# PSeitz/veloci

Hardware: AMD Instinct MI355X
Metric: queries/sec, 3-term AND on 100M-doc index (p50 latency and HBM fraction alongside) (higher is better)
Workload: dtype u32 doc ids + f16->f32 scores

## Files before the change

### veloci_amd/csrc/capi.cpp

```cpp
#include <chrono>
#include <thread>
#include <cstdio>
#include <cstdlib>
#include <cstring>

#include "../../include/veloci_amd.h"
#include <functional>
#include <future>

#include <dlfcn.h>
#include <unistd.h>

#include "engine.hpp"
#include "text.hpp"

using namespace vq;
using vqreq::Request;
using vqreq::VelociError;

namespace {
thread_local std::string g_err;

int fail(int code, const std::string& msg) {
    g_err = msg;
// ... 60 lines not shown
        for (size_t i = 0; i < kv.second.size(); ++i) {
            if (i) s += ',';
            vqjson::escape_to(s, kv.second[i]);
        }
        s += ']';
    }
    s += '}';
}

static void why_found_info_json(std::string& s, const Result& R) {
    s += '{';
    bool first = true;
    for (auto& [anchor, fields] : R.why_found_info) {
        if (!first) s += ',';
        first = false;
        s += '"' + std::to_string(anchor) + "\":";
        why_found_terms_json(s, fields);
    }
    s += '}';
}

namespace {
void dump_f32(std::string& s, float f) {
    uint32_t b;
    std::memcpy(&b, &f, 4);
    s += std::to_string(b);
}
template <class T, class F>
void dump_opt(std::string& s, const std::optional<T>& v, F f) {
    if (v) f(s, *v);
    else s += "null";
}
void dump_usize(std::string& s, size_t v) { s += std::to_string(v); }
void dump_bool(std::string& s, bool v) { s += v ? "true" : "false"; }
void dump_str(std::string& s, const std::string& v) { vqjson::escape_to(s, v); }
void dump_boost_part(std::string& s, const vqreq::RequestBoostPart& b) {
    static const char* const names[] = {"Log2", "Log10", "Multiply", "Add", "Replace"};
    s += "{\"path\":";
    dump_str(s, b.path);
    s += ",\"boost_fun\":";
    if (b.boost_fun) s += std::string("\"") + names[int(*b.boost_fun)] + "\"";
    else s += "null";
    s += ",\"param\":";
    dump_opt(s, b.param, dump_f32);
    s += ",\"skip_when_score\":";
    if (b.skip_when_score) {
        s += '[';
        for (size_t i = 0; i < b.skip_when_score->size(); ++i) {
            if (i) s += ',';
            dump_f32(s, (*b.skip_when_score)[i]);
        }
        s += ']';
    } else s += "null";
    s += ",\"expression\":";
    dump_opt(s, b.expression, dump_str);
    s += '}';
}
void dump_boost_list(std::string& s, const std::optional<std::vector<vqreq::RequestBoostPart>>& v) {
    if (!v) {
        s += "null";
        return;
    }
    s += '[';
    for (size_t i = 0; i < v->size(); ++i) {
        if (i) s += ',';
        dump_boost_part(s, (*v)[i]);
    }
    s += ']';
}
void dump_options(std::string& s, const std::optional<vqreq::SearchRequestOptions>& o) {
    if (!o) {
        s += "null";
        return;
    }
    s += "{\"explain\":";
    dump_bool(s, o->explain);
    s += ",\"top\":";
    dump_opt(s, o->top, dump_usize);
    s += ",\"skip\":";
    dump_opt(s, o->skip, dump_usize);
    s += ",\"boost\":";
    dump_boost_list(s, o->boost);
    s += '}';
}
void dump_part(std::string& s, const vqreq::RequestSearchPart& p) {
    s += "{\"path\":";
    dump_str(s, p.path);
    s += ",\"terms\":[";
    for (size_t i = 0; i < p.terms.size(); ++i) {
        if (i) s += ',';
        dump_str(s, p.terms[i]);
    }
    s += "],\"levenshtein_distance\":";
    if (p.levenshtein_distance) s += std::to_string(*p.levenshtein_distance);
    else s += "null";
    s += ",\"starts_with\":";
    dump_bool(s, p.starts_with);
    s += ",\"is_regex\":";
    dump_bool(s, p.is_regex);
    s += ",\"token_value\":";
    if (p.token_value) dump_boost_part(s, *p.token_value);
    else s += "null";
    s += ",\"boost\":";
    dump_opt(s, p.boost, dump_f32);
    s += ",\"ignore_case\":";
    dump_opt(s, p.ignore_case, dump_bool);
    s += ",\"snippet\":";
    dump_opt(s, p.snippet, dump_bool);
    s += ",\"snippet_info\":";
    dump_bool(s, p.has_snippet_info);
    s += ",\"top\":";
    dump_opt(s, p.top, dump_usize);
    s += ",\"skip\":";
    dump_opt(s, p.skip, dump_usize);
    s += ",\"options\":";
    dump_options(s, p.options);
    s += '}';
}
void dump_search_request(std::string& s, const vqreq::SearchRequest& r) {
    if (r.kind == vqreq::SearchRequest::Search) {
        s += "{\"search\":";
        dump_part(s, r.part);
        s += '}';
        return;
    }
    s += r.kind == vqreq::SearchRequest::Or ? "{\"or\":{\"queries\":[" : "{\"and\":{\"queries\":[";
    for (size_t i = 0; i < r.tree.queries.size(); ++i) {
        if (i) s += ',';
        dump_search_request(s, r.tree.queries[i]);
    }
    s += "],\"options\":";
    dump_options(s, r.tree.options);
    s += "}}";
}
void dump_parts(std::string& s, const std::optional<std::vector<vqreq::RequestSearchPart>>& v) {
    if (!v) {
        s += "null";
        return;
    }
    s += '[';
    for (size_t i = 0; i < v->size(); ++i) {
        if (i) s += ',';
        dump_part(s, (*v)[i]);
    }
    s += ']';
}
}

extern "C" {

const char* vq_last_error(void) { return g_err.c_str(); }
const char* vq_version(void) { return "veloci_amd 0.3 (gfx950)"; }
uint32_t vq_debug_div100_mismatches(void) { return vq::debug_div100_mismatches(); }
uint64_t vq_index_speculative_reruns(const vq_index* index) { return index ? index->idx->or_reruns.load() : 0; }
int vq_debug_facet_select(const uint32_t* hist, uint32_t num_values, uint32_t top, uint32_t misalign, uint32_t* out_values, uint32_t* out_counts) {
    if (!hist || !out_values || !out_counts) return -1;
    return vq::debug_facet_select(hist, num_values, top, misalign, out_values, out_counts);
}

vq_index_builder* vq_index_builder_new(uint32_t num_anchors, uint32_t doc_lo, uint32_t doc_hi) {
    auto* b = new vq_index_builder();
    b->b.num_anchors = num_anchors;
    b->b.doc_lo = doc_lo;
    b->b.doc_hi = doc_hi;
    return b;
}
void vq_index_builder_free(vq_index_builder* b) { delete b; }

int vq_index_add_fst(vq_index_builder* b, const char* path, uint32_t num_terms, const uint8_t* term_bytes, const uint64_t* term_offsets) {
    return guard([&] {
        if (!b || !path || (num_terms && (!term_bytes || !term_offsets))) throw VelociError(VQ_ERR_INVALID_ARGUMENT, "vq_index_add_fst: null argument");
        HostFst f;
        f.terms.reserve(num_terms);
        for (uint32_t i = 0; i < num_terms; ++i) {
            f.terms.emplace_back(reinterpret_cast<const char*>(term_bytes) + term_offsets[i], size_t(term_offsets[i + 1] - term_offsets[i]));
            if (i && !(f.terms[i - 1] < f.terms[i])) throw VelociError(VQ_ERR_INVALID_ARGUMENT, std::string("terms must be bytewise sorted and unique: ") + path);
        }
        b->b.fst[path] = std::move(f);
    });
}

int vq_index_add_token_to_anchor_score(vq_index_builder* b, const char* path, uint32_t num_tokens, const uint64_t* offsets, const uint32_t* anchors,
                                       const uint32_t* scores, const uint64_t* global_lens) {
    return guard([&] {
        if (!b || !path || !offsets) throw VelociError(VQ_ERR_INVALID_ARGUMENT, "vq_index_add_token_to_anchor_score: null argument");
        HostPostings p;
        p.offsets.assign(offsets, offsets + num_tokens + 1);
        const uint64_t n = offsets[num_tokens];
        if (n && (!anchors || !scores)) throw VelociError(VQ_ERR_INVALID_ARGUMENT, "vq_index_add_token_to_anchor_score: null arrays");
        p.anchors.resize(n);
        p.scores.resize(n);
        const size_t piece = size_t(1) << 24;
        parallel_for((n + piece - 1) / piece, host_threads(), [&](size_t i) {
            const size_t off = i * piece, m = std::min<size_t>(piece, n - off);
            std::memcpy(p.anchors.data() + off, anchors + off, m * 4);
            std::memcpy(p.scores.data() + off, scores + off, m * 4);
        });
        parallel_for(num_tokens, host_threads(), [&](size_t t) {
            for (uint64_t i = offsets[t] + 1; i < offsets[t + 1]; ++i)
                if (!(anchors[i - 1] < anchors[i])) throw VelociError(VQ_ERR_INVALID_ARGUMENT, std::string("posting lists must be ascending and unique: ") + path);
        });
        if (global_lens) p.global_lens.assign(global_lens, global_lens + num_tokens);
        b->b.postings[path] = std::move(p);
    });
}

int vq_index_add_key_value_store(vq_index_builder* b, const char* path, uint32_t key_base, uint32_t num_keys, const uint64_t* offsets,
                                 const uint32_t* values) {
    return guard([&] {
        if (!b || !path || !offsets) throw VelociError(VQ_ERR_INVALID_ARGUMENT, "vq_index_add_key_value_store: null argument");
        HostKV k;
        k.key_base = key_base;
        k.offsets.assign(offsets, offsets + num_keys + 1);
        const uint64_t n = offsets[num_keys];
        if (n && !values) throw VelociError(VQ_ERR_INVALID_ARGUMENT, "vq_index_add_key_value_store: null values");
        k.values.assign(values, values + n);
        b->b.kv[path] = std::move(k);
    });
}

int vq_index_add_phrase_pair_to_anchor(vq_index_builder* b, const char* path, uint64_t num_pairs, const uint32_t* t1, const uint32_t* t2,
                                       const uint64_t* offsets, const uint32_t* anchors) {
    return guard([&] {
        if (!b || !path || !offsets) throw VelociError(VQ_ERR_INVALID_ARGUMENT, "vq_index_add_phrase_pair_to_anchor: null argument");
        HostPhrase p;
        p.t1.assign(t1, t1 + num_pairs);
        p.t2.assign(t2, t2 + num_pairs);
        p.offsets.assign(offsets, offsets + num_pairs + 1);
        p.anchors.assign(anchors, anchors + offsets[num_pairs]);
        b->b.phrase[path] = std::move(p);
    });
}

int vq_index_add_boost(vq_index_builder* b, const char* path, uint32_t key_base, uint32_t num_keys, const uint8_t* present, const uint32_t* value_bits) {
    return guard([&] {
        if (!b || !path || (num_keys && !value_bits)) throw VelociError(VQ_ERR_INVALID_ARGUMENT, "vq_index_add_boost: null argument");
        HostBoost h;
        h.key_base = key_base;
        if (present) h.present.assign(present, present + num_keys);
        h.bits.assign(value_bits, value_bits + num_keys);
        b->b.boost[path] = std::move(h);
    });
}

int vq_index_set_column_meta(vq_index_builder* b, const char* field, int is_anchor_identity_column, int tokenize) {
    return guard([&] {
        if (!b || !field) throw VelociError(VQ_ERR_INVALID_ARGUMENT, "vq_index_set_column_meta: null argument");
        ColumnMeta m;
        m.is_anchor_identity_column = is_anchor_identity_column != 0;
        m.tokenize = tokenize != 0;
        b->b.columns[field] = m;
    });
}

int vq_index_build(vq_index_builder* b, int device, vq_index** out) {
    return guard([&] {
        if (!b || !out) throw VelociError(VQ_ERR_INVALID_ARGUMENT, "vq_index_build: null argument");
        *out = nullptr;
        auto idx = build_index(b->b, device);
        auto* h = new vq_index();
        h->idx = std::move(idx);
        *out = h;
    });
}
void vq_index_free(vq_index* i) { delete i; }

int vq_index_set_stream(vq_index* i, void* hip_stream) {
    return guard([&] {
        if (!i) throw VelociError(VQ_ERR_INVALID_ARGUMENT, "vq_index_set_stream: null index");
        std::vector<std::unique_lock<std::mutex>> quiet;
        for (auto& w : i->idx->ws) quiet.emplace_back(w.mu);
        i->idx->stream = hip_stream ? static_cast<hipStream_t>(hip_stream) : i->idx->own_stream;
        i->idx->fin_stream = hip_stream ? static_cast<hipStream_t>(hip_stream) : i->idx->own_fin_stream;
    });
}
int vq_index_set_streams(vq_index* i, void* scan_stream, void* finish_stream) {
    return guard([&] {
        if (!i) throw VelociError(VQ_ERR_INVALID_ARGUMENT, "vq_index_set_streams: null index");
        if (!scan_stream || !finish_stream) throw VelociError(VQ_ERR_INVALID_ARGUMENT, "vq_index_set_streams: null stream (vq_index_set_stream(index, NULL) restores the index's own)");
        std::vector<std::unique_lock<std::mutex>> quiet;
        for (auto& w : i->idx->ws) quiet.emplace_back(w.mu);
        i->idx->stream = static_cast<hipStream_t>(scan_stream);
        i->idx->fin_stream = static_cast<hipStream_t>(finish_stream);
    });
}
int vq_index_set_allreduce(vq_index* i, vq_allreduce_u64_fn fn, void* ctx) {
    return guard([&] {
        if (!i) throw VelociError(VQ_ERR_INVALID_ARGUMENT, "vq_index_set_allreduce: null index");
        std::vector<std::unique_lock<std::mutex>> quiet;
        for (auto& w : i->idx->ws) quiet.emplace_back(w.mu);
        i->idx->allreduce_fn = fn;
        i->idx->allreduce_ctx = ctx;
    });
}
uint64_t vq_index_device_bytes(const vq_index* i) { return i ? i->idx->device_bytes : 0; }

int vq_request_parse(const char* json, size_t len, vq_request** out) {
    return guard([&] {
        if (!json || !out) throw VelociError(VQ_ERR_INVALID_ARGUMENT, "vq_request_parse: null argument");
        *out = nullptr;
        auto* r = new vq_request();
        try {
            r->req = vqreq::request_from_json_text(json, len);
        } catch (...) {
            delete r;
            throw;
// ... 956 lines not shown
```

### veloci_amd/csrc/compile.cpp

```cpp
#include <algorithm>
#include <cmath>
#include <cstdlib>
#include <cstring>
#include <regex>
#include <set>

#include "engine.hpp"
#include "text.hpp"

namespace vq {
std::atomic<uint64_t> g_compile_ns[16];

using namespace vqreq;

namespace {

bool ends_with(const std::string& s, const char* suf) {
    size_t n = std::strlen(suf);
    return s.size() >= n && std::memcmp(s.data() + s.size() - n, suf, n) == 0;
}

[[noreturn]] void unsupported(const std::string& what) {
    throw VelociError(ERR_UNSUPPORTED, "unsupported on the MI355X query path: " + what);
}
// ... 531 lines not shown
        std::vector<uint32_t> all;
        for (uint32_t id : l.hits_ids) {
            const uint32_t *b, *e;
            if (t2a.host_row(id, &b, &e)) all.insert(all.end(), b, e);
        }
        std::sort(all.begin(), all.end());
        if (!with_multiplicity) all.erase(std::unique(all.begin(), all.end()), all.end());
        return layered_inline(all);
    }
    std::vector<uint32_t> layered_inline(const std::vector<uint32_t>& sorted_ids) {
        std::vector<std::vector<uint32_t>> layers;
        for (size_t i = 0; i < sorted_ids.size();) {
            size_t j = i;
            while (j < sorted_ids.size() && sorted_ids[j] == sorted_ids[i]) ++j;
            const size_t mult = j - i;
            if (layers.size() < mult) layers.resize(mult);
            for (size_t m = 0; m < mult; ++m) layers[m].push_back(sorted_ids[i]);
            i = j;
        }
        std::vector<uint32_t> out;
        for (auto& l : layers) out.push_back(add_inline_list(std::move(l)));
        return out;
    }

    static size_t union_min() {
        static const size_t v = std::getenv("VQ_UNION_MIN") ? size_t(std::atoi(std::getenv("VQ_UNION_MIN"))) : 4;
        return v;
    }
    static bool has_wide_and(const SearchRequest& r) {
        if (r.kind == SearchRequest::Search) return false;
        if (r.kind == SearchRequest::And && r.tree.queries.size() >= 3) return true;
        for (auto& q : r.tree.queries)
            if (has_wide_and(q)) return true;
        return false;
    }

    void push_op(std::vector<DOp>& ops, const DOp& op, uint32_t& sp) {
        if (ops.size() >= size_t(kMaxOps)) unsupported("query tree with more than " + std::to_string(kMaxOps) + " nodes");
        ops.push_back(op);
        if (op.kind != OP_LEAF) sp -= op.nchild;
        ++sp;
        max_depth = std::max(max_depth, sp);
        if (sp > uint32_t(kStackDepth)) unsupported("query tree deeper than the evaluation stack");
    }

    std::string leaf_union_key(const Leaf& l) {
        const PostingStore& ps = posting_store(l);
        size_t nonempty = 0;
        for (auto& [tid, score] : l.hits_scores)
            if (tid < ps.num_tokens && ps.global_len[tid]) ++nonempty;
        if (!(nonempty > union_min() || (nonempty > 1 && req.search_req && has_wide_and(*req.search_req)))) return std::string();
        return "u|" + l.path + "|" + (l.key.empty() ? l.part->key() : l.key);
    }

    NodeInfo compile_leaf_scores(const SearchRequest& r, Leaf& l, std::vector<DOp>& ops, uint32_t& sp) {
        std::vector<Leaf*> one{&l};
        return compile_leaf_lists(r.part.terms[0], one, ops, sp);
    }

    NodeInfo compile_leaf_lists(const std::string& label, const std::vector<Leaf*>& members, std::vector<DOp>& ops, uint32_t& sp) {
        PhaseTimer pt(3);
        NodeInfo info;
        DOp op{};
        op.kind = OP_LEAF;
        op.list_begin = uint16_t(cq.lists.size());
        info.label = label;
        struct Entry {
            const PostingStore* ps;
            uint32_t tid;
            float score;
        };
        std::vector<Entry> entries;
        entries.reserve(4);
        info.cover.reserve(4);
        for (Leaf* l : members) {
            const PostingStore& ps = posting_store(*l);
            for (auto& [tid, score] : l->hits_scores)
                if (tid < ps.num_tokens) entries.push_back({&ps, tid, score});
        }
        size_t nonempty = 0;
        for (auto& e : entries)
            if (e.ps->global_len[e.tid]) ++nonempty;
        uint32_t count = 0;
        if (nonempty > union_min() || (nonempty > 1 && req.search_req && has_wide_and(*req.search_req))) {
            std::string ukey;
            if (members.size() == 1) ukey = leaf_union_key(*members[0]);
            else {
                ukey = "u|fused";
                for (Leaf* l : members) ukey += "|" + l->path + "|" + (l->key.empty() ? l->part->key() : l->key);
            }
            const UnionJob* done = nullptr;
            if (unions) {
                auto it = unions->find(ukey);
                if (it != unions->end()) done = &it->second;
            }
            info.glen = 0;
            if (!done) {
                UnionJob job;
                job.key = ukey;
                for (auto& e : entries)
                    if (e.ps->global_len[e.tid]) {
                        job.terms.push_back(UnionJob::Term{e.ps, e.tid, e.score});
                        job.input_postings += e.ps->len[e.tid];
                    }
                cq.union_requests.push_back(std::move(job));
                info.len_known = true;
            } else {
                if (done->len) {
                    HList h;
                    h.d_docs = done->d_docs;
                    h.d_scores = reinterpret_cast<const uint16_t*>(done->d_vals);
                    h.len = done->len;
                    h.global_len = done->global_len;
                    h.flags = LIST_HAS_SCORES | LIST_F32;
                    h.term_score = 1.0f;
                    h.max_value = done->max_value;
                    uint32_t li = add_list(h);
                    info.cover.push_back(li);
                    info.cover_len += h.len;
                    count = 1;
                }
                cq.algorithmic_bytes += 6ull * done->input_postings + 8ull * done->len;
                info.glen = done->global_len;
                info.len_known = !req.filter && idx.can_sum_over_shards();
            }
            op.list_count = uint16_t(count);
            push_op(ops, op, sp);
            info.emitted = true;
            return info;
        }
        uint32_t with_entries = 0;
        for (auto& e : entries) {
            const PostingStore& ps = *e.ps;
            if (ps.global_len[e.tid]) ++with_entries;
            if (ps.len[e.tid] == 0) continue;
            HList h;
            h.d_docs = ps.docs.as<uint32_t>() + ps.start[e.tid];
            h.d_scores = ps.scores.as<uint16_t>() + ps.start[e.tid];
            h.len = ps.len[e.tid];
            h.global_len = ps.global_len[e.tid];
            h.flags = LIST_HAS_SCORES;
            h.term_score = e.score;
            h.max_raw = ps.max_raw[e.tid];
            if (!ps.bm_start.empty() && ps.bm_start[e.tid] >= 0) {
                h.flags |= LIST_BITMAP;
                h.d_bitmap = ps.bitmaps.as<uint32_t>() + ps.bm_start[e.tid];
                h.d_rank_dir = ps.rank_dir.as<uint32_t>() + ps.rd_start[e.tid];
            }
            if (!ps.td_start.empty() && ps.td_start[e.tid] >= 0) h.d_tile_dir = ps.tile_dir.as<uint32_t>() + ps.td_start[e.tid];
            if (!ps.pk_start.empty() && ps.pk_start[e.tid] >= 0) {
                h.d_cov32 = ps.cov32.as<uint32_t>() + uint64_t(ps.pk_start[e.tid]) * 8;
                h.d_gdir = ps.gdir.as<uint32_t>() + ps.gd_start[e.tid];
                if (ps.ak_start[e.tid] >= 0) h.d_arr16 = ps.arr16.as<uint16_t>() + uint64_t(ps.ak_start[e.tid]) * 8;
            }
            uint32_t li = add_list(h);
            info.cover.push_back(li);
            info.cover_len += h.len;
            cq.algorithmic_bytes += 6ull * h.len;
            ++count;
        }
        op.list_count = uint16_t(count);
        info.len_known = with_entries <= 1 && !req.filter;
        info.glen = 0;
        for (auto& e : entries) info.glen += e.ps->global_len[e.tid];
        push_op(ops, op, sp);
        info.emitted = true;
        return info;
    }

    void fill_boost_params(DColBoost& cb, const RequestBoostPart& b) {
        cb.fun = b.boost_fun ? int32_t(*b.boost_fun) : BF_NONE;
        cb.param = b.param.value_or(0.0f);
        if (b.skip_when_score) {
            if (b.skip_when_score->size() > size_t(kMaxSkipWhen)) unsupported("more than 4 skip_when_score values");
            cb.nskip = uint32_t(b.skip_when_score->size());
            for (size_t i = 0; i < b.skip_when_score->size(); ++i) cb.skip[i] = (*b.skip_when_score)[i];
        }
        cb.expr_op = EX_NONE;
        if (b.expression) parse_expression(*b.expression, cb);
    }

    std::vector<uint32_t> boost_1n_text_ids(const RequestSearchPart& part, Leaf& l) {
        std::vector<uint32_t> ids;
        auto cit = idx.columns.find(part.path);
        const bool tokenized = cit != idx.columns.end() && cit->second.tokenize;
        if (tokenized) {
            const KVStore& t2t = kv_store(l.path + TOKENS_TO_TEXT_ID);
            for (auto& h : l.hits_scores) {
                const uint32_t *rb, *re;
                if (t2t.host_row(h.first, &rb, &re)) ids.insert(ids.end(), rb, re);
                else ids.push_back(h.first);
            }
            sort_unique_u32(ids);
        } else ids = l.hits_ids;
        return ids;
    }
    std::vector<std::pair<uint32_t, float>> resolve_boost_1n(const RequestSearchPart& part, Leaf& l, const RequestBoostPart& b) {
        PhaseTimer pt(1);
        std::vector<uint32_t> value_ids;
        {
            PhaseTimer gather(6);
            const std::vector<uint32_t> ids = boost_1n_text_ids(part, l);
            const KVStore& to_parent = kv_store(l.path + VALUE_ID_TO_PARENT);
            for (uint32_t id : ids) {
                const uint32_t *rb, *re;
                if (to_parent.host_row(id, &rb, &re)) value_ids.insert(value_ids.end(), rb, re);
            }
        }
        {
            PhaseTimer sort(7);
            sort_unique_u32(value_ids);
        }
        PhaseTimer pairs_timer(8);
        auto bit = idx.boost.find(b.path + BOOST_VALID_TO_VALUE);
        if (bit == idx.boost.end()) throw VelociError(ERR_INDEX_NOT_FOUND, "Did not found path in indices " + b.path + BOOST_VALID_TO_VALUE);
        const KVStore& to_anchor = kv_store(b.path + VALUE_ID_TO_ANCHOR);
        std::vector<std::pair<uint32_t, float>> pairs;
        pairs.reserve(value_ids.size());
        for (uint32_t vid : value_ids) {
            float v;
            if (!bit->second.host_value(vid, &v)) continue;
            const uint32_t *rb, *re;
            if (to_anchor.host_row(vid, &rb, &re)) pairs.push_back({*rb, v});
        }
        return pairs;
    }

    void emit_boost_1n(const RequestSearchPart& part, Leaf& l, const RequestBoostPart& b, std::vector<DOp>& ops, uint32_t& sp) {
        PhaseTimer pt(2);
        const std::string cache_key = (l.key.empty() ? part.key() : l.key) + "|" + b.path;
        auto emit_layer = [&](const HList& h) {
            const uint32_t li = add_list(h);
            cq.algorithmic_bytes += 8ull * h.len;
            DColBoost cb{};
            fill_boost_params(cb, b);
            cb.nskip = 0;
            cq.leaf_cols.push_back(cb);
            DOp op{};
            op.kind = OP_BOOST1N;
            op.nchild = 1;
            op.list_begin = uint16_t(li);
            op.list_count = 1;
            op.child_slot[0] = uint8_t(cq.leaf_cols.size() - 1);
            push_op(ops, op, sp);
        };
        static const bool device_on = std::getenv("VQ_BOOST1N_DEVICE") != nullptr;
        if (boost_cache && device_on) {
            const std::string to_parent = l.path + VALUE_ID_TO_PARENT, to_anchor = b.path + VALUE_ID_TO_ANCHOR, col = b.path + BOOST_VALID_TO_VALUE;
            auto kp = idx.kv.find(to_parent), ka = idx.kv.find(to_anchor);
            const bool staged = kp != idx.kv.end() && ka != idx.kv.end() && kp->second.value_csr && ka->second.value_csr && idx.boost.count(col);
            if (staged && !boost_cache->device) {
                Boost1nJob job;
                job.key = cache_key;
                job.to_parent_path = to_parent;
                job.to_anchor_path = to_anchor;
                job.boost_path = col;
                job.text_ids = boost_1n_text_ids(part, l);
                cq.boost1n_requests.push_back(std::move(job));
                return;
            }
            if (staged) {
                auto it = boost_cache->device->find(cache_key);
                if (it != boost_cache->device->end() && it->second.done) {
                    const Boost1nJob& job = it->second;
                    if (!job.ascending) unsupported("1:n field boost whose value ids are not in anchor order (" + b.path + ")");
                    if (!job.several) {
                        HList h;
                        h.d_docs = job.d_docs;
                        h.d_scores = reinterpret_cast<const uint16_t*>(job.d_vals);
                        h.len = job.len;
                        h.global_len = job.total;
                        h.flags = LIST_HAS_SCORES | LIST_F32;
                        h.term_score = 1.0f;
                        emit_layer(h);
                        return;
                    }
                }
            }
        }
        std::shared_ptr<Boost1nEntry> entry = boost_cache ? boost_cache->entry(cache_key) : std::make_shared<Boost1nEntry>();
        auto make_layers = [&](const std::vector<std::vector<std::pair<uint32_t, float>>>& layers) {
            auto out = std::make_shared<std::vector<Boost1nEntry::Layer>>();
            for (auto& layer : layers) {
                Boost1nEntry::Layer L;
                L.global_len = layer.size();
                L.docs.reserve(layer.size());
                L.vals.reserve(layer.size());
                for (auto& pr : layer)
                    if (pr.first >= idx.doc_lo && pr.first < idx.doc_hi) {
                        L.docs.push_back(pr.first);
                        L.vals.push_back(pr.second);
                    }
                out->push_back(std::move(L));
            }
            return out;
        };
        std::call_once(entry->resolved, [&] {
            entry->pairs = resolve_boost_1n(part, l, b);
            PhaseTimer order_check(9);
            const auto& pairs = entry->pairs;
            for (size_t i = 1; i < pairs.size(); ++i) {
                if (pairs[i].first < pairs[i - 1].first) entry->ascending = false;
                entry->several = entry->several || pairs[i].first == pairs[i - 1].first;
            }
            if (!entry->ascending) return;
            if (!entry->several) entry->layers = make_layers({pairs});
// ... 1157 lines not shown
                        for (uint32_t e = 0; e < cq.lists.size(); ++e)
                            if (cq.lists[e].d_docs == h.d_docs && cq.lists[e].inline_idx < 0 && cq.lists[e].len == h.len) {
                                li = e;
                                break;
                            }
                        if (li == UINT32_MAX) {
                            li = add_list(h);
                            cq.algorithmic_bytes += 4ull * h.len;
                        }
                        cq.loc_idx.push_back(uint16_t(li));
                        ++count;
                    }
                lf.list_count = uint16_t(count);
                cq.locf.push_back(lf);
            }

        if (req.facets)
            for (auto& fr : *req.facets) {
                std::vector<std::string> steps = get_steps_to_anchor(fr.field);
                std::string store_path;
                if (steps.size() == 1) store_path = steps.front() + PARENT_TO_VALUE_ID;
                else if (idx.kv.count(steps.back() + ANCHOR_TO_TEXT_ID)) store_path = steps.back() + ANCHOR_TO_TEXT_ID;
                const KVStore& kv = store_path.empty() ? idx.composed_facet(steps) : kv_store(store_path);
                if (!kv.facet_csr) unsupported("facet source " + store_path + " is not staged as an anchor-keyed CSR");
                auto dit = idx.dict.find(steps.back());
                if (dit == idx.dict.end()) throw VelociError(ERR_FST_NOT_FOUND, "fst not found loaded in indices " + steps.back() + " ");
                DFacet f{};
                f.offsets = kv.csr_off.as<uint64_t>();
                f.values = kv.csr_values.as<uint32_t>();
                f.direct = kv.csr_direct.p ? kv.csr_direct.as<uint32_t>() : nullptr;
                f.key_base = kv.csr_key_base;
                f.num_keys = kv.csr_num_keys;
                f.num_values = std::max<uint32_t>(uint32_t(dit->second.terms.size()), kv.csr_num_keys ? kv.csr_max_value + 1 : 0);
                const uint64_t want = fr.top ? std::min<uint64_t>(*fr.top, f.num_values) : f.num_values;
                f.top = want > uint64_t(kMaxTopK) ? 0u : uint32_t(want);
                cq.facets.push_back(f);
                FacetOut fo;
                fo.field = fr.field;
                fo.dict_path = steps.back();
                fo.top = f.top;
                fo.host_top = want > uint64_t(kMaxTopK) ? uint32_t(want) : 0u;
                fo.num_values = f.num_values;
                cq.facet_out.push_back(fo);
                cq.algorithmic_bytes += 4ull * f.num_values;
            }
        cq.algorithmic_bytes += 8ull * cq.top_k;

        if (label_wanted) {
            if (maybe_reqs.empty() && count_reqs.empty()) unsupported("OR over an operand whose term label is only known at run time (set_op.rs:143,439)");
            if (!idx.can_sum_over_shards())
                unsupported("OR over an AND whose label follows run-time result sizes, on a sharded index without vq_index_set_allreduce");
            count_reqs.insert(count_reqs.end(), maybe_reqs.begin(), maybe_reqs.end());
        }
        if (2 * count_reqs.size() + 1 > 256) unsupported("more than 127 AND operands whose sizes must be measured first");
        build_presence_program();
        if (!count_reqs.empty())
            for (auto& l : cq.lists) l.flags |= LIST_COVER;
        {
            const size_t n = cq.ops.size();
            auto is_leaf1 = [&](const DOp& o) {
                return o.kind == OP_LEAF && o.list_count == 1 && (cq.lists[o.list_begin].flags & LIST_HAS_SCORES) && !(cq.lists[o.list_begin].flags & LIST_F32);
            };
            if (n == 1 && is_leaf1(cq.ops[0])) cq.simple_n = 1;
            else if (n >= 3 && n <= 5 && cq.ops[n - 1].kind != OP_LEAF && cq.ops[n - 1].nchild == n - 1) {
                bool ok = true;
                for (size_t i = 0; i + 1 < n; ++i) ok = ok && is_leaf1(cq.ops[i]);
                if (ok) cq.simple_n = uint32_t(n - 1);
            }
            if (cq.simple_n > 1 && cq.ops[n - 1].kind == OP_OR && cq.ops[n - 1].nslots == cq.simple_n) {
                DOp& root = cq.ops[n - 1];
                std::vector<std::pair<uint8_t, DOp>> leaves;
                for (uint32_t k = 0; k < cq.simple_n; ++k) leaves.push_back({root.child_slot[k], cq.ops[k]});
                std::stable_sort(leaves.begin(), leaves.end(), [](auto& x, auto& y) { return x.first < y.first; });
                for (uint32_t k = 0; k < cq.simple_n; ++k) {
                    cq.ops[k] = leaves[k].second;
                    root.child_slot[k] = leaves[k].first;
                }
            }
        }

        {
            static const bool force_generic = std::getenv("VQ_FORCE_GENERIC") != nullptr;
            const bool pure = cq.simple_n && count_reqs.empty() && cq.fops.empty() && cq.groups.empty() && cq.tboosts.empty() && cq.cols.empty() && cq.locf.empty() &&
                              cq.facets.empty() && uint64_t(idx.doc_hi) - idx.doc_lo >= 65536;
            if (pure && !force_generic) {
                uint32_t f = 1u << 17;
                static const bool no_probe = std::getenv("VQ_NO_PROBE") != nullptr;
                static const uint64_t probe_min_docs = std::getenv("VQ_PROBE_MIN_DOCS") ? uint64_t(std::atoll(std::getenv("VQ_PROBE_MIN_DOCS"))) : 40'000'000ull;
                bool probe = !no_probe && cq.simple_n >= 2 && cq.ops[cq.simple_n].kind == OP_AND && uint64_t(idx.doc_hi) - idx.doc_lo >= probe_min_docs;
                uint32_t arr_mask = 0;
                if (probe) {
                    static const bool no_arr = std::getenv("VQ_PROBE_NO_ARR") != nullptr;
                    uint32_t covers = 0;
                    for (uint32_t k = 0; k < cq.simple_n; ++k) {
                        const HList& l = cq.lists[cq.ops[k].list_begin];
                        if (l.flags & LIST_COVER) {
                            ++covers;
                            probe = probe && l.d_cov32;
                        } else {
                            const bool arr = l.d_arr16 && !no_arr && (!(l.flags & LIST_BITMAP) || uint64_t(l.len) * 16 < uint64_t(idx.doc_hi) - idx.doc_lo);
                            if (arr) arr_mask |= 1u << k;
                            probe = probe && (arr || (l.flags & LIST_BITMAP));
                        }
                    }
                    probe = probe && covers == 1;
                }
                static const bool no_probe_or = std::getenv("VQ_NO_PROBE_OR") != nullptr;
                uint32_t or_cover = UINT32_MAX;
                if (!probe && !no_probe && !no_probe_or && !req.exact_routes_only && cq.top_k >= 1 && cq.simple_n >= 2 && cq.simple_n <= 3 && cq.ops[cq.simple_n].kind == OP_OR &&
                    cq.ops[cq.simple_n].nslots == cq.simple_n && !idx.sharded() && !(idx.comm && idx.comm->nranks > 1) && uint64_t(idx.doc_hi) - idx.doc_lo >= probe_min_docs) {
                    for (uint32_t k = 0; k < cq.simple_n; ++k) {
                        const HList& l = cq.lists[cq.ops[k].list_begin];
                        if (l.d_cov32 && (or_cover == UINT32_MAX || l.len < cq.lists[cq.ops[or_cover].list_begin].len)) or_cover = k;
                    }
                    double sum = 0.0, cnt = 0.0;
                    for (uint32_t k = 0; k < cq.simple_n && or_cover != UINT32_MAX; ++k) {
                        if (k == or_cover) continue;
                        const HList& l = cq.lists[cq.ops[k].list_begin];
                        if (!(l.flags & LIST_BITMAP) || (l.flags & LIST_F32) || l.max_raw >= 0x7C00 || !(l.term_score >= 0.0f)) {
                            or_cover = UINT32_MAX;
                            break;
                        }
                        const uint16_t h = l.max_raw;
                        const int e = (h >> 10) & 31, m = h & 1023;
                        const double a = e ? std::ldexp(1.0 + m / 1024.0, e - 15) : std::ldexp(m / 1024.0, -14);
                        const double v = double(l.term_score) * (a / 100.0);
                        if (v >= 0.00001 * (1.0 - 1e-5)) cnt += 1.0;
                        sum += v;
                    }
                    if (or_cover != UINT32_MAX) {
                        const HList& c = cq.lists[cq.ops[or_cover].list_begin];
                        if (!(c.term_score > 0.0f) || c.max_raw >= 0x7C00) or_cover = UINT32_MAX;
                        else {
                            const double b = sum * cnt * cnt * (1.0 + 1e-5);
                            cq.or_skip_bound = b < 3.0e38 ? float(b) : std::numeric_limits<float>::infinity();
                            if (cq.or_skip_bound < float(b)) cq.or_skip_bound = std::nextafter(cq.or_skip_bound, std::numeric_limits<float>::infinity());
                            probe = true;
                        }
                    }
                }
                const bool or_probe = or_cover != UINT32_MAX && probe;
                bool seq = false;
                for (uint32_t k = 0; k < cq.simple_n && !probe; ++k) {
                    const HList& l = cq.lists[cq.ops[k].list_begin];
                    if ((l.flags & LIST_COVER) && (l.flags & LIST_BITMAP)) seq = true;
                }
                if (seq) f |= 1u << 16;
                if (probe) {
                    f |= 1u << 25 | arr_mask << 12 | (or_probe ? 1u << 27 : 0u);
                    cq.probe = DProbe{};
                    for (uint32_t k = 0; k < cq.simple_n; ++k) {
                        const HList& l = cq.lists[cq.ops[k].list_begin];
                        cq.probe.leaf[k] = DProbeLeaf{l.d_cov32, l.d_arr16, l.d_gdir};
                    }
                }
                static const bool ring = std::getenv("VQ_RING") != nullptr && std::atoi(std::getenv("VQ_RING")) != 0;
                if (probe && ring && !arr_mask && !or_probe && cq.top_k >= 1 && cq.top_k <= kPoolMaxK) f |= 1u << 26;
                for (uint32_t k = 0; k < cq.simple_n; ++k) {
                    const HList& l = cq.lists[cq.ops[k].list_begin];
                    const bool cover = or_probe ? k == or_cover : (l.flags & LIST_COVER) != 0;
                    if (cover) f |= 1u << (8 + k);
                    if ((l.flags & LIST_BITMAP) && (seq || !cover) && !((arr_mask >> k) & 1u)) f |= 1u << k;
                    if (uint64_t(l.len) * 8192 >= 200 * (uint64_t(idx.doc_hi) - idx.doc_lo)) f |= 1u << (20 + k);
                }
                static const bool no_union_cov = std::getenv("VQ_NO_UNION_COV") != nullptr;
                if (cq.simple_n == 1 && !no_union_cov) {
                    const HList& l = cq.lists[cq.ops[0].list_begin];
                    if (l.d_cov32 && l.d_gdir && l.d_tile_dir && l.term_score > 0.0f && !(l.flags & LIST_F32) && l.inline_idx < 0) {
                        f |= 1u << 28;
                        cq.probe = DProbe{};
                        cq.probe.leaf[0] = DProbeLeaf{l.d_cov32, l.d_arr16, l.d_gdir};
                    }
                }
                cq.simple_flags = f;
            }
        }

        {
            static const bool off = std::getenv("VQ_FORCE_GENERIC") != nullptr || std::getenv("VQ_NO_LEAF_F32") != nullptr;
            if (!off && !cq.simple_flags && count_reqs.empty() && cq.ops.size() == 1 && cq.ops[0].kind == OP_LEAF && cq.ops[0].list_count == 1 &&
                (cq.lists[cq.ops[0].list_begin].flags & LIST_F32) && cq.fops.empty() && cq.groups.empty() && cq.tboosts.empty() && cq.cols.empty() && cq.locf.empty() &&
                cq.facets.empty())
                cq.simple_flags = 1u << 19;
        }
        if (!cq.simple_flags) detect_rich_simple();
        if (!cq.simple_flags) detect_wide();
        if (!cq.simple_flags || ((cq.simple_flags >> 24) & 1u)) compute_prune_table();
        if (!cq.simple_flags && count_reqs.empty()) {
            bool dense_cover = false;
            for (auto& l : cq.lists) dense_cover = dense_cover || ((l.flags & LIST_COVER) && (l.flags & LIST_BITMAP));
            if (dense_cover) {
                cq.seq_tiles = 1;
                for (auto& l : cq.lists)
                    if (l.flags & LIST_BITMAP) l.flags &= ~uint32_t(LIST_COVER);
            }
        }

        const uint32_t L = std::max<uint32_t>(uint32_t(cq.lists.size()), 1);
        const uint64_t range = uint64_t(idx.doc_hi) - idx.doc_lo;
        static const uint32_t ww_max = [] {
            const char* e = std::getenv("VQ_TILE_WORDS_MAX");
            uint32_t v = e ? uint32_t(std::atoi(e)) : 256u;
            uint32_t p2 = 64;
            while (p2 < v && p2 < 2048) p2 <<= 1;
            return p2;
        }();
        static const size_t var_budget = [] {
            const char* e = std::getenv("VQ_TILE_LDS_KB");
            return size_t(e ? std::atoi(e) : 12) * 1024;
        }();
        static const uint64_t span_env = [] {
            const char* e = std::getenv("VQ_SPAN_POSTINGS");
            return uint64_t(e ? std::atoll(e) : 0);
        }();
        const bool and_like = ((cq.simple_flags >> 18) & 1u) || (cq.simple_flags && cq.simple_n > 1 && cq.ops.back().kind == OP_AND);
        const bool wide_like = (cq.simple_flags >> 24) & 1u;
        const bool probe_like = (cq.simple_flags >> 25) & 1u;
        const uint64_t probe_span = std::min<uint64_t>(std::max<uint64_t>(range / 96, 131072), 1048576);
        const bool or_like = cq.simple_flags && !((cq.simple_flags >> 18) & 1u) && !wide_like && !probe_like && cq.simple_n > 1 && cq.ops.back().kind == OP_OR;
        const uint64_t span_postings = span_env ? span_env : (probe_like ? probe_span : and_like ? 131072 : wide_like ? 589824 : (or_like && range >= 50'000'000ull) ? 524288 : 262144);
        uint32_t ww = ww_max;
        const size_t TL = size_t(L) + cq.n_temps;
        while (ww > 64 && (size_t(ww) + TL * ww + size_t(L) * ww / 2) * 4 > var_budget) ww >>= 1;
        if ((size_t(ww) + TL * ww + size_t(L) * ww / 2) * 4 > 96 * 1024) unsupported("too many lists for the LDS tile");
        const uint64_t cover_len = std::max<uint64_t>(root.cover_len, 1);
        if (cover_len * (uint64_t(ww) << 5) / std::max<uint64_t>(range, 1) < 64) {
            const uint64_t want = std::max<uint64_t>(range / cover_len, 2048);
            while (ww > 64 && (uint64_t(ww) << 5) / 2 >= want) ww >>= 1;
        }
        if (cq.simple_flags) ww = 256;
        cq.tile_words = ww;
        cq.stack_depth = std::max<uint32_t>(max_depth, 1);
        uint64_t spans = (cq.total_len + span_postings - 1) / span_postings;
        static const uint64_t facet_span = [] {
            const char* e = std::getenv("VQ_FACET_SPAN_POSTINGS");
            return uint64_t(e ? std::atoll(e) : 4096);
        }();
        if (!cq.facets.empty()) spans = (cq.total_len + facet_span - 1) / facet_span;
        const uint64_t tiles = std::max<uint64_t>((range + (uint64_t(ww) << 5) - 1) / (uint64_t(ww) << 5), 1);
        {
            uint64_t cover_len = 0;
            for (auto& l : cq.lists)
                if (l.flags & LIST_COVER) cover_len += l.len;
            const uint64_t visited = std::max<uint64_t>(std::min<uint64_t>(cover_len, tiles), 1);
            if (!cq.simple_flags && cq.total_len / visited < 1024) spans = std::max<uint64_t>(spans, visited / 16);
            if (((cq.simple_flags >> 18) & 1u) && cq.total_len / visited < 1024) spans = std::max<uint64_t>(spans, visited / 64);
        }
        if ((cq.simple_flags >> 26) & 1u) {
            static const uint64_t ring_tiles = [] {
                const char* e = std::getenv("VQ_RING_SPAN_TILES");
                return uint64_t(e ? std::max(1, std::atoi(e)) : 64);
            }();
            const uint64_t ptiles = std::max<uint64_t>((range + (1u << kProbeTileShift) - 1) >> kProbeTileShift, 1);
            spans = (ptiles + ring_tiles - 1) / ring_tiles;
        }
        spans = std::min<uint64_t>(spans, tiles);
        spans = std::min<uint64_t>(std::max<uint64_t>(spans, 1), 4096);
        cq.n_spans = uint32_t(spans);
        if ((cq.simple_flags >> 19) & 1u) {
            const uint64_t len = cq.lists[cq.ops[0].list_begin].len;
            cq.n_spans = uint32_t(std::min<uint64_t>(std::max<uint64_t>(len / (cq.facets.empty() ? 16384 : 4096), 1), 4096));
        }
        cq.max_spans = uint32_t(std::min<uint64_t>(std::max<uint64_t>(tiles, 1), 4096));
        if ((cq.simple_flags >> 19) & 1u) cq.max_spans = uint32_t(std::min<uint64_t>(std::max<uint64_t>(cq.lists[cq.ops[0].list_begin].len / 64, 1), 4096));
        compute_layout_bytes(root.cover_len);
    }

    void compute_layout_bytes(uint64_t cover_len) {
        const uint64_t range = uint64_t(idx.doc_hi) - idx.doc_lo;
        const bool simple = cq.simple_flags != 0;
        const bool wide = (cq.simple_flags >> 24) & 1u;
        const uint64_t tile_docs = wide ? 8192 : ((cq.simple_flags >> 25) & 1u) ? (1u << kProbeTileShift) : simple ? 16384 : uint64_t(cq.tile_words) << 5;
        const uint64_t tiles = std::max<uint64_t>((range + tile_docs - 1) / tile_docs, 1);
        const bool seq = wide ? cq.wide.seq != 0 : simple ? ((cq.simple_flags >> 16) & 1u) : cq.seq_tiles != 0;
        const uint64_t visited = seq ? tiles : std::min<uint64_t>(std::max<uint64_t>(cover_len, 1), tiles);
        auto bitmap_cost = [&]() { return visited * (tile_docs / 8 + 4); };
        uint64_t b = 8ull * cq.top_k;
        if ((cq.simple_flags >> 19) & 1u) b += 8ull * cq.lists[cq.ops[0].list_begin].len;
        else if (simple && !((cq.simple_flags >> 18) & 1u) && cq.simple_n == 1 && std::getenv("VQ_NO_UNION") == nullptr)
            b += (((cq.simple_flags >> 28) & 1u) ? 4ull : 6ull) * cq.lists[cq.ops[0].list_begin].len;
        else if (wide) {
            for (uint32_t k = 0; k < cq.wide.n_leaves; ++k) b += ((cq.wide.bitmap_mask >> k) & 1u) ? bitmap_cost() : 4ull * cq.lists[cq.wide.leaf_list[k]].len;
        } else if ((cq.simple_flags >> 25) & 1u) {
            for (uint32_t k = 0; k < cq.simple_n; ++k) {
                const uint64_t len = cq.lists[cq.ops[k].list_begin].len;
                b += ((cq.simple_flags >> k) & 1u) ? visited * (tile_docs / 8 + 4 * (tile_docs >> kRankShift)) : ((cq.simple_flags >> (12 + k)) & 1u) ? 2ull * len : 4ull * len;
            }
        } else if (simple) {
            std::vector<bool> seen(cq.lists.size(), false);
            const bool rich = (cq.simple_flags >> 18) & 1u;
            for (uint32_t k = 0; k < cq.simple_n; ++k) {
                const uint32_t li = rich ? cq.simple2.leaf_list[k] : cq.ops[k].list_begin;
                seen[li] = true;
                b += ((cq.simple_flags >> k) & 1u) ? bitmap_cost() : 4ull * cq.lists[li].len;
            }
            for (uint32_t li = 0; li < cq.lists.size(); ++li)
                if (!seen[li]) b += 4ull * cq.lists[li].len;
        } else {
            for (auto& l : cq.lists) {
                const bool as_bitmap = (l.flags & LIST_BITMAP) && !(l.flags & LIST_COVER);
                b += as_bitmap ? bitmap_cost() : 4ull * l.len;
            }
        }
        for (auto& f : cq.facets) b += 4ull * f.num_values;
        cq.layout_bytes = b;
    }
// ... 371 lines not shown
```

### veloci_amd/csrc/engine.hpp

```cpp
#pragma once
#include <hip/hip_runtime.h>

#include <atomic>
#include <cmath>
#include <chrono>
#include <cstdint>
#include <map>
#include <limits>
#include <memory>
#include <thread>
#include <functional>
#include <condition_variable>
#include <mutex>
#include <string>
#include <unordered_map>
#include <vector>

#include "device_types.hpp"
#include "kernels.hpp"
#include "request.hpp"
#include "hostpool.hpp"

namespace vq {

// ... 120 lines not shown
    T* as() const { return reinterpret_cast<T*>(p); }
};

struct Dictionary {
    std::vector<std::string> terms;
    std::unordered_map<std::string, std::vector<uint32_t>> lower_map;
    uint32_t char_bytes = 2;
    bool low_exact = true;
    DevBuf d_off;
    DevBuf d_raw;
    DevBuf d_low;
};

struct Index;
struct PostingStore;
struct FuzzyProbe {
    std::string key;
    std::string path;
    std::vector<uint32_t> query;
    uint32_t max_d = 0;
    bool transposition = false, prefix = false, ci = true;
    std::vector<uint32_t> matches;
    std::vector<float> scores;
    std::string lower_term;
    uint32_t lev = 0;
    bool check_prefix = false;
    int status = 0;
    std::string error;
};
using FuzzyTable = std::map<std::string, FuzzyProbe>;
std::string fuzzy_key(const vqreq::RequestSearchPart& p);
bool needs_dictionary_scan(const vqreq::RequestSearchPart& p);
void collect_fuzzy_probes(const Index& idx, const vqreq::Request& req, FuzzyTable& table);
struct Workspace;
void run_fuzzy_probes(const Index& idx, Workspace& ws, FuzzyTable& table, hipStream_t st);
void score_fuzzy_probe(const Index& idx, FuzzyProbe& probe);
float default_score_for_distance_host(uint8_t distance, bool prefix_matches);
size_t debug_sort_unique(uint32_t* ids, size_t n);
struct SuggestEntry {
    std::string text;
    float score;
    uint32_t term_id;
};
std::vector<SuggestEntry> suggest_part(const Index& idx, const vqreq::RequestSearchPart& part, const FuzzyTable* fuzzy);
void collect_suggest_probes(const Index& idx, const vqreq::Request& req, FuzzyTable& table);
std::optional<std::string> highlight_text(const std::string& text, const std::vector<std::string>& terms, const vqreq::SnippetInfo& opt, bool tokenized);
vqreq::Request page_request_after(const vqreq::Request& request, float score, uint32_t id);
std::vector<SuggestEntry> highlight_part(const Index& idx, const vqreq::RequestSearchPart& part, const FuzzyTable* fuzzy);
std::vector<SuggestEntry> run_highlight(const Index& idx, vqreq::RequestSearchPart part);
std::vector<SuggestEntry> run_suggest(const Index& idx, const vqreq::Request& req);

struct UnionJob {
    std::string key;
    struct Term {
        const PostingStore* store;
        uint32_t token;
        float score;
    };
    std::vector<Term> terms;
    const uint32_t* d_docs = nullptr;
    const float* d_vals = nullptr;
    float max_value = std::numeric_limits<float>::infinity();
    uint32_t len = 0;
    uint64_t global_len = 0;
    uint64_t input_postings = 0;
};
using UnionTable = std::map<std::string, UnionJob>;
struct RangeJob {
    std::string key;
    std::string store_path;
    std::vector<uint32_t> tokens;
    std::string union_key;
    std::shared_ptr<const std::vector<uint32_t>> anchors;
    std::vector<uint64_t> counts;
};
using RangeTable = std::map<std::string, RangeJob>;
struct Boost1nEntry {
    struct Layer {
        std::vector<uint32_t> docs;
        std::vector<float> vals;
        uint64_t global_len = 0;
    };
    std::once_flag resolved, layered;
    std::vector<std::pair<uint32_t, float>> pairs;
    bool ascending = true, several = false;
    std::vector<uint32_t> anchors;
    std::shared_ptr<const std::vector<Layer>> layers;
};
struct Boost1nCache {
    static constexpr size_t kShards = 64;
    struct Shard {
        std::mutex mu;
        std::unordered_map<std::string, std::shared_ptr<Boost1nEntry>> map;
    } shard[kShards];
    std::shared_ptr<Boost1nEntry> entry(const std::string& key) {
        Shard& sh = shard[std::hash<std::string>{}(key) % kShards];
        std::lock_guard<std::mutex> g(sh.mu);
        auto& slot = sh.map[key];
        if (!slot) slot = std::make_shared<Boost1nEntry>();
        return slot;
    }
    const std::map<std::string, struct Boost1nJob>* device = nullptr;
};
struct LocalityJob {
    std::string key;
    std::string t2t_path, t2a_path;
    std::vector<uint32_t> tokens;
    const uint32_t* d_docs = nullptr;
    const float* d_vals = nullptr;
    uint32_t len = 0;
};
using LocalityTable = std::map<std::string, LocalityJob>;
struct Boost1nJob {
    std::string key;
    std::string to_parent_path, to_anchor_path, boost_path;
    std::vector<uint32_t> text_ids;
    const uint32_t* d_docs = nullptr;
    const float* d_vals = nullptr;
    uint32_t len = 0;
    uint32_t total = 0;
    bool ascending = true;
    bool several = false;
    bool done = false;
};
using Boost1nTable = std::map<std::string, Boost1nJob>;
constexpr int kStatusNeedsUnion = -1;
constexpr int kStatusNeedsCounts = -2;
constexpr int kStatusNeedsRanges = -3;

struct QueryCounts {
    bool has_filter = false;
    uint64_t filter_count = 0;
    std::map<uint32_t, std::pair<uint64_t, uint64_t>> nodes;
};

struct PostingStore {
    uint32_t num_tokens = 0;
    std::vector<uint64_t> start;
    std::vector<uint32_t> len;
    std::vector<uint64_t> global_len;
    std::vector<uint16_t> max_raw;
    DevBuf docs;
    DevBuf scores;
    uint64_t total_padded = 0;
    std::vector<int64_t> bm_start;
    std::vector<int64_t> rd_start;
    DevBuf bitmaps;
    DevBuf rank_dir;
    std::vector<int64_t> td_start;
    DevBuf tile_dir;
    std::vector<int64_t> pk_start;
    std::vector<int64_t> ak_start;
    std::vector<int64_t> gd_start;
    DevBuf cov32, arr16, gdir;
};

struct KVStore {
    uint32_t key_base = 0, num_keys = 0;
    std::vector<uint64_t> host_off;
    std::vector<uint32_t> host_values;
    bool list_rows = false;
    bool rows_sorted_unique = true;
    bool rows_equal_postings = false;
    std::vector<uint64_t> start;
    std::vector<uint32_t> len;
    DevBuf values;
    DevBuf d_row_start, d_row_len;
    bool text_csr = false;
    DevBuf d_text_vals;
    bool value_csr = false;
    DevBuf d_csr_off;
    bool facet_csr = false;
    uint32_t csr_key_base = 0, csr_num_keys = 0;
    uint32_t csr_max_value = 0;
    DevBuf csr_direct;
    DevBuf csr_off;
    DevBuf csr_values;

    bool host_row(uint64_t key, const uint32_t** b, const uint32_t** e) const {
        if (key < key_base) return false;
        uint64_t r = key - key_base;
        if (r >= num_keys || host_off[r] == host_off[r + 1]) return false;
        *b = host_values.data() + host_off[r];
        *e = host_values.data() + host_off[r + 1];
        return true;
    }
};

struct PhraseStore {
    std::vector<std::pair<uint32_t, uint32_t>> keys;
    std::vector<uint64_t> start;
    std::vector<uint32_t> len;
    DevBuf anchors;
};

struct BoostColumn {
    uint32_t key_base = 0, num_keys = 0;
    bool has_present = false;
    float vmin = 0.0f, vmax = 0.0f;
    bool any_value = false, has_nan = false;
    DevBuf values;
    DevBuf present;
    std::vector<uint32_t> host_bits;
    std::vector<uint8_t> host_present;
    bool host_value(uint64_t key, float* out) const {
        if (key < key_base || key - key_base >= host_bits.size()) return false;
        const size_t r = size_t(key - key_base);
        if (!host_present.empty() && !host_present[r]) return false;
        std::memcpy(out, &host_bits[r], 4);
        return true;
    }
};

struct PinnedBuf {
    void* p = nullptr;
    size_t bytes = 0;
    PinnedBuf() = default;
    PinnedBuf(const PinnedBuf&) = delete;
    PinnedBuf& operator=(const PinnedBuf&) = delete;
    ~PinnedBuf();
    void ensure(size_t n);
    template <class T>
    T* as() const { return reinterpret_cast<T*>(p); }
};

constexpr int kWorkspaces = 4;

enum KernelId : int {
    K_DICT_SCAN = 0, K_UNION_COUNT, K_UNION_WRITE, K_RANGE_HITS, K_COUNT_PREPASS, K_SCAN_LEAF_F32, K_SCAN_RICH, K_SCAN_RING, K_SCAN_PROBE, K_SCAN_AND, K_SCAN_SIMPLE, K_SCAN_UNION,
    K_SCAN_WIDE, K_TILE_SCAN, K_MERGE_SPANS, K_FINALIZE, K_FACET_SELECT, K_LOCALITY, K_BOOST1N, K_COUNT_
};
extern const char* const kKernelNames[K_COUNT_];

struct TimedLaunch {
    int kernel;
    uint32_t ev_begin, ev_end;
    uint64_t layout_bytes, algorithmic_bytes, queries;
};

struct Workspace {
    std::mutex mu;
    std::atomic<bool> pinned{false};
    std::vector<hipEvent_t> ev_pool;
    uint32_t ev_used = 0;
    std::vector<TimedLaunch> timed;
    hipEvent_t ev_done = nullptr;
    PinnedBuf h_up, h_down;
    DevBuf d_up;
    DevBuf d_span_keys;
    DevBuf d_partial;
    DevBuf d_down;
    DevBuf d_union_docs[2], d_union_vals[2], d_union_max, d_union_meta;
    DevBuf d_loc_a, d_loc_b, d_loc_pairs_a, d_loc_pairs_b, d_loc_meta, d_loc_tmp, d_loc_docs, d_loc_vals;
    DevBuf d_b1n_a, d_b1n_b, d_b1n_meta, d_b1n_tmp, d_b1n_docs, d_b1n_vals;
    DevBuf d_probe_desc, d_probe_counts, d_probe_ids;
};

struct KernelProfile {
    double ms = 0;
    uint64_t launches = 0;
    uint64_t layout_bytes = 0;
    uint64_t algorithmic_bytes = 0;
    uint64_t gathered_bytes = 0;
    uint64_t queries = 0;
};
struct Profile {
    bool enabled = false;
    KernelProfile k[K_COUNT_];
    uint64_t batches = 0;
};
struct LaunchTimer {
    Workspace* ws = nullptr;
    hipStream_t st = nullptr;
    size_t slot = 0;
    LaunchTimer(bool on, Workspace& w, hipStream_t s, int kernel, uint64_t layout_bytes = 0, uint64_t algorithmic_bytes = 0, uint64_t queries = 0);
    ~LaunchTimer();
    LaunchTimer(const LaunchTimer&) = delete;
    LaunchTimer& operator=(const LaunchTimer&) = delete;
};


struct ShardComm {
    int nranks = 1, rank = 0;
    void* nccl = nullptr;
    int (*allgather)(void* ctx, const void* local, void* gathered, size_t bytes_per_rank, void* stream) = nullptr;
    int (*allreduce_u32)(void* ctx, void* inout, size_t count, void* stream) = nullptr;
    void* ctx = nullptr;
    hipStream_t stream = nullptr;
    hipEvent_t ev_scan[2] = {nullptr, nullptr}, ev_xchg[2] = {nullptr, nullptr}, ev_fin[2] = {nullptr, nullptr};
    void* unmerged = nullptr;
    int live = 0;
    DevBuf gathered[2];
    DevBuf red;
    bool busy[2] = {false, false};
    std::string failed;
    std::mutex mu;
    ~ShardComm();
};

struct Index {
    int device = 0;
    int (*allreduce_fn)(void*, uint64_t*, size_t) = nullptr;
    void* allreduce_ctx = nullptr;
    bool sharded() const { return doc_lo != 0 || doc_hi != num_anchors; }
    bool can_sum_over_shards() const { return !sharded() || allreduce_fn != nullptr; }
    void sum_over_shards(std::vector<uint64_t>& v) const {
        if (!sharded() || v.empty()) return;
        if (!allreduce_fn || allreduce_fn(allreduce_ctx, v.data(), v.size()) != 0) throw vqreq::VelociError(vqreq::ERR_DEVICE, "all-reduce over the shards failed");
    }
    mutable std::atomic<uint64_t> or_reruns{0};
    mutable std::unique_ptr<HostPool> pool;
    mutable std::mutex pool_mu;
    uint32_t num_anchors = 0, doc_lo = 0, doc_hi = 0;
    uint32_t bitmap_base = 0;
    uint64_t bitmap_words = 0;
    std::map<std::string, Dictionary> dict;
    std::map<std::string, PostingStore> postings;
    std::map<std::string, KVStore> kv;
    std::map<std::string, PhraseStore> phrase;
    std::map<std::string, BoostColumn> boost;
    std::map<std::string, ColumnMeta> columns;
    uint64_t device_bytes = 0;
    mutable std::mutex composed_mu;
    mutable std::map<std::string, std::unique_ptr<KVStore>> composed_facets;
    const KVStore& composed_facet(const std::vector<std::string>& steps) const;
    hipStream_t own_stream = nullptr, own_fin_stream = nullptr;
    hipStream_t pre_stream = nullptr;
    hipStream_t stream = nullptr;
    hipStream_t fin_stream = nullptr;
    mutable std::mutex profile_mutex;
    mutable Profile profile;
    mutable Workspace ws[kWorkspaces];
    mutable std::atomic<uint32_t> next_ws{0};
    mutable DevBuf arena;
    static constexpr size_t kArenaBytes = 64ull << 20;
    mutable std::unique_ptr<ShardComm> comm;
    ~Index();
    bool is_anchor_identity(const std::string& textindex_path) const;
};

std::unique_ptr<Index> build_index(const IndexBuilder& b, int device);

struct HList {
    const uint32_t* d_docs = nullptr;
    const uint16_t* d_scores = nullptr;
    uint32_t len = 0;
    uint32_t flags = 0;
    float term_score = 0.f;
    uint16_t max_raw = 0x7C00;
    float max_value = std::numeric_limits<float>::infinity();
    uint64_t global_len = 0;
    const uint32_t* d_bitmap = nullptr;
    const uint32_t* d_rank_dir = nullptr;
    const uint32_t* d_tile_dir = nullptr;
    const uint32_t* d_cov32 = nullptr;
    const uint16_t* d_arr16 = nullptr;
    const uint32_t* d_gdir = nullptr;
    int inline_idx = -1;
    int inline_val_idx = -1;
};

struct FacetOut {
    std::string field;
    std::string dict_path;
    uint32_t top = 10;
    uint32_t num_values = 0;
    uint32_t host_top = 0;
};

struct ExplainRec {
    enum Kind : uint8_t { Boost, MaxTokenToTextId, TermToAnchor, LevenshteinScore, OrSumOverDistinctTerms } kind = Boost;
    float a = 0.0f, b = 0.0f, c = 0.0f;
    uint32_t term_id = 0;
    std::string text;
};
using ExplainRecs = std::vector<ExplainRec>;
struct ExplainNode {
    uint32_t kind = 0;
    int op = -1;
    std::vector<int> children;
    std::vector<uint16_t> order;
    uint32_t list_begin = 0, list_count = 0;
    std::vector<uint32_t> list_term;
    std::map<uint32_t, ExplainRecs> term_records;
};
using WhyFoundPlan = std::map<std::string, std::vector<uint32_t>>;
struct ExplainPlan {
    std::vector<ExplainNode> nodes;
    int root = -1;
    std::vector<ExList> lists;
    std::vector<ExOp> ops;
    std::vector<uint16_t> aux;
    std::vector<DColBoost> cols;
};

struct CompiledQuery {
    size_t blob_bytes = 0, desc_bytes = 0;
    int status = 0;
    std::shared_ptr<const ExplainPlan> explain_plan;
    std::shared_ptr<const WhyFoundPlan> why_found_plan;
    std::string error;
    std::vector<RangeJob> range_requests;
    std::vector<UnionJob> union_requests;
    std::vector<LocalityJob> locality_requests;
    std::vector<Boost1nJob> boost1n_requests;
    std::vector<uint32_t> count_nodes;
    uint32_t n_counts = 0;
    std::vector<HList> lists;
    std::vector<std::vector<uint32_t>> inline_lists;
    std::vector<std::vector<float>> inline_vals;
    std::vector<DColBoost> leaf_cols;
    uint32_t seq_tiles = 0;
    uint32_t prune_n = 0;
    uint64_t prune_mask = 0;
    uint32_t prune_gbits[16] = {};
    uint32_t n_top_cols = 0;
    std::vector<DOp> ops, fops;
    std::vector<DPresOp> pres;
    std::vector<uint16_t> pres_in;
    uint32_t n_temps = 0;
    uint32_t simple_n = 0;
    uint32_t simple_flags = 0;
    std::vector<DGroup> groups;
    std::vector<DTermBoost> tboosts;
    std::vector<DColBoost> cols;
    std::vector<DLocField> locf;
    std::vector<uint16_t> loc_idx;
    DSimple2 simple2{};
    DWide wide{};
    DProbe probe{};
    std::vector<DFacet> facets;
    std::vector<FacetOut> facet_out;
    std::map<std::string, std::vector<std::string>> why_found_terms;
    uint32_t top = 10, skip = 0, top_k = 10;
    uint64_t total_len = 0;
    uint64_t algorithmic_bytes = 0;
    uint64_t layout_bytes = 0;
    uint64_t key_upper = ~0ull;
    float or_skip_bound = std::numeric_limits<float>::quiet_NaN();
    bool deep = false;
    uint32_t tile_words = 0, n_spans = 1, stack_depth = 1;
    uint32_t max_spans = 1;
};

CompiledQuery compile_query(const Index& idx, const vqreq::Request& req, const FuzzyTable* fuzzy = nullptr, const UnionTable* unions = nullptr,
                            const QueryCounts* counts = nullptr, const RangeTable* ranges = nullptr, Boost1nCache* boost_cache = nullptr,
                            const LocalityTable* localities = nullptr);
void run_locality_jobs(const Index& idx, Workspace& ws, LocalityTable& table, hipStream_t st);
void run_boost1n_jobs(const Index& idx, Workspace& ws, Boost1nTable& table, hipStream_t st);
void run_range_jobs(const Index& idx, Workspace& ws, RangeTable& table, const UnionTable& unions, hipStream_t st);
void run_union_jobs(const Index& idx, Workspace& ws, UnionTable& table, hipStream_t st);
struct Result;
void complete_explain_requests(const Index& idx, std::vector<std::unique_ptr<Result>>& results, std::vector<int>& status, std::vector<std::string>& errors);
void complete_why_found_requests(const Index& idx, std::vector<std::unique_ptr<Result>>& results, std::vector<int>& status, std::vector<std::string>& errors);
bool request_wants_explain(const vqreq::Request& req);
std::string explain_records_json(const ExplainRecs& records);
void complete_deep_requests(const Index& idx, const vqreq::Request* const* reqs, size_t n, std::vector<std::unique_ptr<Result>>& results,
                            std::vector<int>& status, std::vector<std::string>& errors);

struct ResultFacet {
    std::string field;
    std::vector<std::pair<std::string, uint64_t>> entries;
};
struct Result {
    uint64_t num_hits = 0;
    uint64_t execution_time_ns = 0;
    std::vector<uint32_t> ids;
    std::vector<float> scores;
    std::vector<ResultFacet> facets;
    bool has_facets = false;
    std::map<std::string, std::vector<std::string>> why_found_terms;
    std::shared_ptr<const ExplainPlan> explain_plan;
    std::shared_ptr<const WhyFoundPlan> why_found_plan;
    std::map<uint32_t, std::map<std::string, std::vector<std::string>>> why_found_info;
    bool has_explain = false;
    std::vector<std::pair<bool, ExplainRecs>> explain;
    bool deep = false;
    bool rerun_exact = false;
    mutable std::string json;
};

struct PartialBatch {
    const Index* index = nullptr;
    Workspace* ws = nullptr;
    std::unique_lock<std::mutex> lock;
    bool pinned_ws = false;
    std::vector<CompiledQuery> queries;
    std::vector<uint32_t> slot;
    std::vector<uint8_t> qclass;
    std::vector<FacetJob> facet_jobs;
    uint32_t nq_dev = 0;
    PartialLayout layout{};
    const uint8_t* d_blobs = nullptr;
    const uint32_t* d_blob_off = nullptr;
    const uint32_t* d_span_base = nullptr;
    const FacetJob* d_facet_jobs = nullptr;
    uint8_t* d_partial = nullptr;
    uint32_t total_spans = 0;
    uint32_t n_facet_jobs = 0;
    uint32_t total_facet_out = 0;
    bool profiled = false;
    bool launched = false, finished = false;
    bool merge_launched = false;
    std::chrono::steady_clock::time_point t0;
    void release_workspace();
    std::vector<const vqreq::Request*> reqs;
    ~PartialBatch();
};

std::unique_ptr<PartialBatch> run_partial(const Index& idx, const vqreq::Request* const* reqs, size_t n, int slot = -1, int64_t arena_offset = -1);
void finish_batch(const Index& idx, PartialBatch& pb, const void* gathered_device, uint32_t num_shards, std::vector<std::unique_ptr<Result>>& out,
                  std::vector<int>& status, std::vector<std::string>& errors, size_t shard_stride = 0);
void finish_launch(const Index& idx, PartialBatch& pb, const void* gathered_device, uint32_t num_shards, size_t shard_stride = 0);

}
```

### veloci_amd/csrc/exec.cpp

```cpp
#include <algorithm>
#include <cstdio>
#include <cstdlib>
#include <cstring>
#include <thread>

#include "engine.hpp"

#include "text.hpp"

namespace vq {

using namespace vqreq;

void DevBuf::ensure(size_t n) {
    if (n <= bytes) return;
    size_t want = std::max(n, bytes + bytes / 2);
    alloc(want);
}
PinnedBuf::~PinnedBuf() {
    if (p) (void)hipHostFree(p);
}
void PinnedBuf::ensure(size_t n) {
    if (n <= bytes) return;
    if (p) (void)hipHostFree(p);
// ... 1022 lines not shown
                const std::vector<std::pair<size_t, size_t>> ranges = guided_ranges(again.size(), host_threads(), heavy_first ? 4 * host_threads() : 0);
                host_pool(idx).run(ranges.size(), [&](size_t p) { recompile(ranges[p].first, ranges[p].second); });
            } else recompile(0, again.size());
            std::vector<size_t> still;
            for (size_t i : again)
                if (pb->queries[i].status == kStatusNeedsRanges) still.push_back(i);
            again.swap(still);
        }
    }
    const RangeTable* rangesp = ranges.empty() ? nullptr : &ranges;
    {
        std::vector<size_t> need;
        std::vector<CompiledQuery*> cqs;
        for (size_t i = 0; i < n; ++i)
            if (pb->queries[i].status == kStatusNeedsCounts) {
                need.push_back(i);
                cqs.push_back(&pb->queries[i]);
            }
        if (!need.empty()) {
            std::vector<QueryCounts> counts;
            run_count_queries(idx, ws, cqs, counts, pst);
            if (idx.sharded()) {
                std::vector<uint64_t> flat;
                for (auto& c : counts) {
                    flat.push_back(c.filter_count);
                    for (auto& kv : c.nodes) {
                        flat.push_back(kv.second.first);
                        flat.push_back(kv.second.second);
                    }
                }
                idx.sum_over_shards(flat);
                size_t k = 0;
                for (auto& c : counts) {
                    c.filter_count = flat[k++];
                    for (auto& kv : c.nodes) {
                        kv.second.first = flat[k++];
                        kv.second.second = flat[k++];
                    }
                }
            }
            for (size_t k = 0; k < need.size(); ++k) {
                CompiledQuery& q = pb->queries[need[k]];
                q = compile_query(idx, *reqs[need[k]], fuzzy.empty() ? nullptr : &fuzzy, unions.empty() ? nullptr : &unions, &counts[k], rangesp, &boost_cache,
                                  localities.empty() ? nullptr : &localities);
                if (q.status < 0) {
                    q.status = ERR_UNSUPPORTED;
                    q.error = "unsupported on the MI355X query path: query still needs a pre-pass after the count pre-pass (internal)";
                }
            }
        }
    }
    const double t_compiled = now_ms();
    uint32_t nq = 0;
    uint64_t total_keys = 0, total_hist = 0, total_span_keys = 0, total_spans = 0, blob_bytes = 0;
    uint32_t max_lists = 1, max_ww = 32;
    size_t lds_bytes = 0;
    uint32_t stack_depth = 1;
    std::vector<uint32_t> keys_base, part_keys_off, span_base;
    std::vector<std::vector<uint32_t>> hist_offs, fac_out_offs;
    std::vector<FacetJob> jobs;
    uint32_t fac_out_total = 0;
    {
        static const uint64_t target1 = [] {
            const char* e = std::getenv("VQ_SPAN_TARGET");
            return uint64_t(e ? std::atoll(e) : 2048);
        }();
        const uint64_t target = std::min<uint64_t>(target1 + 64 * uint64_t(n - 1), std::max<uint64_t>(target1, 5120));
        uint64_t have = 0;
        for (size_t i = 0; i < n; ++i)
            if (pb->queries[i].status == 0) have += pb->queries[i].n_spans;
        if (have && have * 3 <= target * 2) {
            const uint64_t f = (target + have - 1) / have;
            for (size_t i = 0; i < n; ++i) {
                CompiledQuery& cq = pb->queries[i];
                if (cq.status == 0) cq.n_spans = uint32_t(std::max<uint64_t>(cq.n_spans, std::min<uint64_t>(uint64_t(cq.n_spans) * f, cq.max_spans)));
            }
        }
        static const bool weighted = std::getenv("VQ_NO_WEIGHTED_SPANS") == nullptr;
        uint64_t total_postings = 0;
        for (size_t i = 0; i < n; ++i)
            if (pb->queries[i].status == 0) total_postings += pb->queries[i].total_len;
        if (weighted && n > 1 && total_postings) {
            const uint64_t per_span = std::max<uint64_t>(total_postings / target, 4096);
            for (size_t i = 0; i < n; ++i) {
                CompiledQuery& cq = pb->queries[i];
                if (cq.status != 0) continue;
                const uint64_t want = std::min<uint64_t>((cq.total_len + per_span - 1) / per_span, cq.max_spans);
                cq.n_spans = uint32_t(std::max<uint64_t>(cq.n_spans, want));
            }
        }
    }
    for (size_t i = 0; i < n; ++i) {
        CompiledQuery& cq = pb->queries[i];
        if (cq.status != 0) continue;
        pb->slot[i] = nq++;
        keys_base.push_back(uint32_t(total_span_keys));
        part_keys_off.push_back(uint32_t(total_keys));
        span_base.push_back(uint32_t(total_spans));
        total_span_keys += uint64_t(cq.n_spans) * cq.top_k;
        total_keys += cq.top_k;
        total_spans += cq.n_spans;
        std::vector<uint32_t> ho, fo;
        for (auto& f : cq.facets) {
            ho.push_back(uint32_t(total_hist));
            fo.push_back(fac_out_total);
            jobs.push_back(FacetJob{uint32_t(total_hist), f.num_values, f.top, fac_out_total});
            total_hist += f.num_values;
            fac_out_total += f.top;
        }
        hist_offs.push_back(std::move(ho));
        fac_out_offs.push_back(std::move(fo));
        if (!cq.blob_bytes) size_blob(cq, idx);
        blob_bytes += cq.blob_bytes;
        max_lists = std::max<uint32_t>(max_lists, uint32_t(cq.lists.size()));
        max_ww = std::max(max_ww, cq.tile_words);
        stack_depth = std::max(stack_depth, cq.stack_depth);
    }
    if (total_span_keys > 0xFFFFFFFFull || total_hist > 0xFFFFFFFFull || total_spans > 0x7FFFFFFFull)
        throw VelociError(ERR_UNSUPPORTED, "batch too large for 32-bit workspace offsets: split the batch");
    span_base.push_back(uint32_t(total_spans));
    pb->nq_dev = nq;
    pb->total_spans = uint32_t(total_spans);
    pb->n_facet_jobs = uint32_t(jobs.size());
    pb->total_facet_out = fac_out_total;
    pb->facet_jobs = jobs;
    const double t_layout = now_ms();

    PartialLayout& lay = pb->layout;
    lay.nq = nq;
    lay.total_keys = total_keys;
    lay.total_hist = total_hist;
    lay.off_hits = 0;
    lay.off_stats = align_up(size_t(nq) * 8, 16);
    lay.off_keys = lay.off_stats + align_up(size_t(nq) * 8, 16);
    lay.off_hist = align_up(lay.off_keys + size_t(total_keys) * 8, 256);
    lay.bytes = align_up(lay.off_hist + size_t(total_hist) * 4, 256);

    const size_t up_blob_off = align_up(blob_bytes, 256);
    const size_t tbl = align_up(size_t(nq + 1) * 4, 256);
    const size_t up_span_base = up_blob_off + tbl;
    const size_t up_qmap_g = up_span_base + tbl;
    const size_t up_span_s = up_qmap_g + tbl;
    const size_t up_qmap_s = up_span_s + tbl;
    const size_t up_span_d = up_qmap_s + tbl;
    const size_t up_qmap_d = up_span_d + tbl;
    const size_t up_span_w = up_qmap_d + tbl;
    const size_t up_qmap_w = up_span_w + tbl;
    const size_t up_span_r = up_qmap_w + tbl;
    const size_t up_qmap_r = up_span_r + tbl;
    const size_t up_span_f = up_qmap_r + tbl;
    const size_t up_qmap_f = up_span_f + tbl;
    const size_t up_span_x = up_qmap_f + tbl;
    const size_t up_qmap_x = up_span_x + tbl;
    const size_t up_span_p = up_qmap_x + tbl;
    const size_t up_qmap_p = up_span_p + tbl;
    const size_t up_qmap_n = up_qmap_p + tbl;
    const size_t up_work_n = up_qmap_n + tbl;
    size_t ring_items_max = 0;
    for (size_t i = 0; i < n; ++i)
        if (pb->queries[i].status == 0 && ((pb->queries[i].simple_flags >> 26) & 1u)) ring_items_max += pb->queries[i].n_spans;
    const size_t up_items_n = up_work_n + 256;
    const size_t up_jobs = up_items_n + align_up(ring_items_max * 4, 256);
    const size_t up_bytes = up_jobs + align_up(jobs.size() * sizeof(FacetJob), 256) + 256;
    ws.h_up.ensure(up_bytes);
    ws.d_up.ensure(up_bytes);
    uint8_t* hup = ws.h_up.as<uint8_t>();
    uint8_t* dup = ws.d_up.as<uint8_t>();
    bool union_has_or = false;
    uint32_t scatter_wide = 0, scatter_simple = 0;
    uint32_t n_simple = 0, n_generic = 0, n_dense = 0, n_wide = 0, n_rich = 0, spans_simple = 0, spans_generic = 0, spans_dense = 0, spans_wide = 0, spans_rich = 0;
    uint32_t scatter_rich = 0;
    bool facets_rich = false;
    uint32_t n_leaf = 0, spans_leaf = 0;
    uint32_t n_xwide = 0, spans_xwide = 0, leaves_xwide = 0, scatter_xwide = 0;
    uint32_t n_probe = 0, spans_probe = 0, nd_probe = 1;
    bool probe_any_and = false, probe_any_or = false;
    uint32_t n_ring = 0, items_ring = 0, nd_ring = 1, ring_spans_each = 0;
    uint64_t cls_layout[K_COUNT_] = {}, cls_algo[K_COUNT_] = {}, cls_q[K_COUNT_] = {};
    {
        size_t off = 0;
        uint32_t* hbo = reinterpret_cast<uint32_t*>(hup + up_blob_off);
        uint32_t qi = 0;
        for (size_t i = 0; i < n; ++i) {
            CompiledQuery& cq = pb->queries[i];
            if (cq.status != 0) continue;
            hbo[qi] = uint32_t(off);
            const size_t packed = pack_blob(cq, idx, hup + off, dup + off, keys_base[qi], part_keys_off[qi], hist_offs[qi], fac_out_offs[qi], nullptr,
                                            pb->profiled ? uint32_t((lay.off_stats - lay.off_hits) / 8 + qi) : 0u);
            if (packed != cq.blob_bytes) throw VelociError(ERR_DEVICE, "query blob changed size between compilation and packing (internal)");
            off += packed;
            ++qi;
        }
        hbo[nq] = uint32_t(off);
        uint32_t* sg = reinterpret_cast<uint32_t*>(hup + up_span_base);
        uint32_t* mg = reinterpret_cast<uint32_t*>(hup + up_qmap_g);
        uint32_t* ss = reinterpret_cast<uint32_t*>(hup + up_span_s);
        uint32_t* ms = reinterpret_cast<uint32_t*>(hup + up_qmap_s);
        uint32_t* sd = reinterpret_cast<uint32_t*>(hup + up_span_d);
        uint32_t* md = reinterpret_cast<uint32_t*>(hup + up_qmap_d);
        uint32_t* sw = reinterpret_cast<uint32_t*>(hup + up_span_w);
        uint32_t* mw = reinterpret_cast<uint32_t*>(hup + up_qmap_w);
        uint32_t* sr = reinterpret_cast<uint32_t*>(hup + up_span_r);
        uint32_t* mr = reinterpret_cast<uint32_t*>(hup + up_qmap_r);
        uint32_t* sf = reinterpret_cast<uint32_t*>(hup + up_span_f);
        uint32_t* mf = reinterpret_cast<uint32_t*>(hup + up_qmap_f);
        uint32_t accf = 0, accx = 0;
        uint32_t* sx = reinterpret_cast<uint32_t*>(hup + up_span_x);
        uint32_t* mx = reinterpret_cast<uint32_t*>(hup + up_qmap_x);
        uint32_t accg = 0, accs = 0, accd = 0, accw = 0, accr = 0, accp = 0;
        uint32_t* sp = reinterpret_cast<uint32_t*>(hup + up_span_p);
        uint32_t* mp = reinterpret_cast<uint32_t*>(hup + up_qmap_p);
        uint32_t* mn = reinterpret_cast<uint32_t*>(hup + up_qmap_n);
        uint32_t ring_max_spans = 0;
        std::vector<uint32_t> ring_ns;
        bool ring_uniform = true;
        std::memset(hup + up_work_n, 0, 256);
        qi = 0;
        for (size_t i = 0; i < n; ++i) {
            const CompiledQuery& cq = pb->queries[i];
            if (cq.status != 0) continue;
            static const bool union_enabled = std::getenv("VQ_NO_UNION") == nullptr;
            static const bool union_or = std::getenv("VQ_UNION_OR") != nullptr;
            const bool rich = (cq.simple_flags >> 18) & 1u;
            const bool dense = !rich && union_enabled && cq.simple_flags && (cq.simple_n == 1 || (union_or && cq.ops.back().kind == OP_OR));
            int kclass;
            if ((cq.simple_flags >> 19) & 1u) {
                kclass = K_SCAN_LEAF_F32;
                sf[n_leaf] = accf;
                mf[n_leaf++] = qi;
                accf += cq.n_spans;
            } else if ((cq.simple_flags >> 24) & 1u) {
                kclass = K_SCAN_WIDE;
                leaves_xwide = std::max<uint32_t>(leaves_xwide, cq.wide.n_leaves);
                scatter_xwide = std::max<uint32_t>(scatter_xwide, cq.wide.n_leaves - uint32_t(__builtin_popcount(cq.wide.bitmap_mask)));
                sx[n_xwide] = accx;
                mx[n_xwide++] = qi;
                accx += cq.n_spans;
            } else if (rich) {
                kclass = K_SCAN_RICH;
                facets_rich = facets_rich || !cq.facets.empty();
                scatter_rich = std::max<uint32_t>(scatter_rich, cq.simple_n - uint32_t(__builtin_popcount(cq.simple_flags & 0xFu)) + cq.simple2.n_side);
                sr[n_rich] = accr;
                mr[n_rich++] = qi;
                accr += cq.n_spans;
            } else if (dense) {
                kclass = K_SCAN_UNION;
                union_has_or = union_has_or || cq.simple_n > 1;
                sd[n_dense] = accd;
                md[n_dense++] = qi;
                accd += cq.n_spans;
            } else if ((cq.simple_flags >> 26) & 1u) {
                kclass = K_SCAN_RING;
                nd_ring = std::max<uint32_t>(nd_ring, cq.simple_n - 1);
                ring_uniform = ring_uniform && (n_ring == 0 || cq.n_spans == ring_max_spans);
                ring_max_spans = std::max(ring_max_spans, cq.n_spans);
                mn[n_ring++] = qi;
                ring_ns.push_back(cq.n_spans);
                items_ring += cq.n_spans;
            } else if ((cq.simple_flags >> 25) & 1u) {
                kclass = K_SCAN_PROBE;
                ((cq.simple_flags >> 27) & 1u ? probe_any_or : probe_any_and) = true;
                nd_probe = std::max<uint32_t>(nd_probe, cq.simple_n - 1);
                sp[n_probe] = accp;
                mp[n_probe++] = qi;
                accp += cq.n_spans;
            } else if (cq.simple_flags && cq.simple_n > 1 && cq.ops.back().kind == OP_AND) {
                kclass = K_SCAN_AND;
                scatter_wide = std::max<uint32_t>(scatter_wide, cq.simple_n - uint32_t(__builtin_popcount(cq.simple_flags & 0xFu)));
                sw[n_wide] = accw;
                mw[n_wide++] = qi;
                accw += cq.n_spans;
            } else if (cq.simple_flags) {
                kclass = K_SCAN_SIMPLE;
                scatter_simple = std::max<uint32_t>(scatter_simple, cq.simple_n - uint32_t(__builtin_popcount(cq.simple_flags & 0xFu)));
                ss[n_simple] = accs;
                ms[n_simple++] = qi;
                accs += cq.n_spans;
            } else {
                kclass = K_TILE_SCAN;
                sg[n_generic] = accg;
                mg[n_generic++] = qi;
                accg += cq.n_spans;
            }
            pb->qclass.push_back(uint8_t(kclass));
            cls_layout[kclass] += cq.layout_bytes;
            cls_algo[kclass] += cq.algorithmic_bytes;
            cls_q[kclass] += 1;
            ++qi;
        }
        sg[n_generic] = accg;
        ss[n_simple] = accs;
        sw[n_wide] = accw;
        spans_wide = accw;
        sr[n_rich] = accr;
        spans_rich = accr;
        sf[n_leaf] = accf;
        spans_leaf = accf;
        sx[n_xwide] = accx;
        spans_xwide = accx;
        sp[n_probe] = accp;
        spans_probe = accp;
        if (n_ring) {
            if (ring_uniform) ring_spans_each = ring_max_spans;
            else {
                uint32_t* it = reinterpret_cast<uint32_t*>(hup + up_items_n);
                uint32_t k = 0;
                for (uint32_t r = 0; r < ring_max_spans; ++r)
                    for (uint32_t j = 0; j < n_ring; ++j)
                        if (r < ring_ns[j]) it[k++] = (j << 12) | r;
            }
        }
        sd[n_dense] = accd;
        spans_generic = accg;
        spans_simple = accs;
        spans_dense = accd;
        if (!jobs.empty()) std::memcpy(hup + up_jobs, jobs.data(), jobs.size() * sizeof(FacetJob));
    }
    pb->d_blobs = dup;
    pb->d_blob_off = reinterpret_cast<const uint32_t*>(dup + up_blob_off);
    pb->d_span_base = reinterpret_cast<const uint32_t*>(dup + up_span_base);
    pb->d_facet_jobs = reinterpret_cast<const FacetJob*>(dup + up_jobs);
    if (nq == 0) return pb;

    const double t_packed = now_ms();
    VQ_HIP(hipMemcpyAsync(dup, hup, up_bytes, hipMemcpyHostToDevice, st));
    ws.d_span_keys.ensure(size_t(total_span_keys) * 8 + 16);
    if (arena_offset >= 0) {
        if (size_t(arena_offset) % 256 || size_t(arena_offset) + lay.bytes > Index::kArenaBytes)
            throw VelociError(ERR_UNSUPPORTED, "partial arena: the step's partials do not fit (" + std::to_string(size_t(arena_offset) + lay.bytes) + " bytes)");
        idx.arena.ensure(Index::kArenaBytes);
        pb->d_partial = idx.arena.as<uint8_t>() + arena_offset;
    } else {
        ws.d_partial.ensure(lay.bytes);
        pb->d_partial = ws.d_partial.as<uint8_t>();
    }
    VQ_HIP(hipMemsetAsync(pb->d_partial, 0, lay.bytes, st));

    uint32_t max_top_k = 1;
    for (size_t i = 0; i < n; ++i)
        if (pb->queries[i].status == 0) max_top_k = std::max(max_top_k, pb->queries[i].top_k);
    uint32_t desc_cap = 0;
    for (size_t i = 0; i < n; ++i)
        if (pb->queries[i].status == 0) {
            desc_cap = std::max(desc_cap, uint32_t(pb->queries[i].desc_bytes));
        }
    desc_cap = uint32_t(align_up(desc_cap, 16));
    bool facets_generic = false;
    static const bool no_facet_cache = std::getenv("VQ_NO_FACET_CACHE") != nullptr;
    for (size_t i = 0; i < n; ++i)
        if (pb->queries[i].status == 0 && !pb->queries[i].simple_flags && !pb->queries[i].facets.empty()) facets_generic = !no_facet_cache;
    if (facets_generic) desc_cap += 2 * 1024 * 4;
    static const uint32_t cand_min = [] {
        const char* e = std::getenv("VQ_CAND_CAP");
        return uint32_t(e ? std::max(32, std::atoi(e)) : 32);
    }();
    uint32_t cand_cap = cand_min;
    while (cand_cap < 2 * max_top_k) cand_cap <<= 1;
    const uint32_t list_table = (std::max<uint32_t>(max_lists, 2) + 1u) & ~1u;
    static const bool tile_queue = std::getenv("VQ_NO_QUEUE") == nullptr;
    for (size_t i = 0; i < n; ++i)
        if (pb->queries[i].status == 0 && !pb->queries[i].simple_flags)
            lds_bytes = std::max(lds_bytes, tile_scan_lds_bytes(uint32_t(pb->queries[i].lists.size()) + pb->queries[i].n_temps, uint32_t(pb->queries[i].lists.size()), pb->queries[i].tile_words, stack_depth, cand_cap, desc_cap, tile_queue && !pb->queries[i].simple_n, list_table));
    if (lds_bytes > 160 * 1024) throw VelociError(ERR_UNSUPPORTED, "LDS tile larger than 160 KiB");
    const bool prof = pb->profiled;
    auto hits_ptr = reinterpret_cast<unsigned long long*>(pb->d_partial + lay.off_hits);
    auto hist_ptr = reinterpret_cast<uint32_t*>(pb->d_partial + lay.off_hist);
    auto keys_ptr = ws.d_span_keys.as<unsigned long long>();
    auto tab = [&](size_t o) { return reinterpret_cast<const uint32_t*>(dup + o); };
    if (spans_leaf) {
        LaunchTimer t(prof, ws, st, K_SCAN_LEAF_F32, cls_layout[K_SCAN_LEAF_F32], cls_algo[K_SCAN_LEAF_F32], cls_q[K_SCAN_LEAF_F32]);
        launch_scan_leaf_f32(st, spans_leaf, pb->d_blobs, pb->d_blob_off, tab(up_span_f), tab(up_qmap_f), n_leaf, cand_cap, keys_ptr, hits_ptr, hist_ptr);
    }
    VQ_HIP(hipGetLastError());
    if (spans_rich) {
        LaunchTimer t(prof, ws, st, K_SCAN_RICH, cls_layout[K_SCAN_RICH], cls_algo[K_SCAN_RICH], cls_q[K_SCAN_RICH]);
        launch_scan_simple(st, true, scatter_rich, spans_rich, pb->d_blobs, pb->d_blob_off, tab(up_span_r), tab(up_qmap_r), n_rich, cand_cap, keys_ptr, hits_ptr, hist_ptr, facets_rich);
    }
    VQ_HIP(hipGetLastError());
    if (items_ring) {
        static const uint32_t cus = [] {
            int dev = 0, v = 0;
            if (hipGetDevice(&dev) != hipSuccess || hipDeviceGetAttribute(&v, hipDeviceAttributeMultiprocessorCount, dev) != hipSuccess || v <= 0) v = 256;
            return uint32_t(v);
        }();
        LaunchTimer t(prof, ws, st, K_SCAN_RING, cls_layout[K_SCAN_RING], cls_algo[K_SCAN_RING], cls_q[K_SCAN_RING]);
        launch_scan_ring(st, nd_ring, cus, pb->d_blobs, pb->d_blob_off, tab(up_qmap_n), n_ring, ring_spans_each, tab(up_items_n), items_ring,
                         reinterpret_cast<uint32_t*>(dup + up_work_n), keys_ptr, hits_ptr);
    }
    VQ_HIP(hipGetLastError());
    if (spans_probe) {
        LaunchTimer t(prof, ws, st, K_SCAN_PROBE, cls_layout[K_SCAN_PROBE], cls_algo[K_SCAN_PROBE], cls_q[K_SCAN_PROBE]);
        launch_scan_probe(st, nd_probe, spans_probe, pb->d_blobs, pb->d_blob_off, tab(up_span_p), tab(up_qmap_p), n_probe, cand_cap, keys_ptr, hits_ptr, probe_any_and, probe_any_or);
    }
    VQ_HIP(hipGetLastError());
    if (spans_wide) {
        LaunchTimer t(prof, ws, st, K_SCAN_AND, cls_layout[K_SCAN_AND], cls_algo[K_SCAN_AND], cls_q[K_SCAN_AND]);
        launch_scan_simple(st, false, scatter_wide, spans_wide, pb->d_blobs, pb->d_blob_off, tab(up_span_w), tab(up_qmap_w), n_wide, cand_cap, keys_ptr, hits_ptr, hist_ptr);
    }
    VQ_HIP(hipGetLastError());
    if (spans_simple) {
        LaunchTimer t(prof, ws, st, K_SCAN_SIMPLE, cls_layout[K_SCAN_SIMPLE], cls_algo[K_SCAN_SIMPLE], cls_q[K_SCAN_SIMPLE]);
        launch_scan_simple(st, false, scatter_simple, spans_simple, pb->d_blobs, pb->d_blob_off, tab(up_span_s), tab(up_qmap_s), n_simple, cand_cap, keys_ptr, hits_ptr, hist_ptr);
    }
    VQ_HIP(hipGetLastError());
    if (spans_dense) {
        LaunchTimer t(prof, ws, st, K_SCAN_UNION, cls_layout[K_SCAN_UNION], cls_algo[K_SCAN_UNION], cls_q[K_SCAN_UNION]);
        launch_scan_union(st, union_has_or, spans_dense, pb->d_blobs, pb->d_blob_off, tab(up_span_d), tab(up_qmap_d), n_dense, cand_cap, keys_ptr, hits_ptr);
    }
    VQ_HIP(hipGetLastError());
    if (spans_xwide) {
        LaunchTimer t(prof, ws, st, K_SCAN_WIDE, cls_layout[K_SCAN_WIDE], cls_algo[K_SCAN_WIDE], cls_q[K_SCAN_WIDE]);
        launch_scan_wide(st, leaves_xwide, scatter_xwide, spans_xwide, pb->d_blobs, pb->d_blob_off, tab(up_span_x), tab(up_qmap_x), n_xwide, cand_cap, keys_ptr, hits_ptr);
    }
    VQ_HIP(hipGetLastError());
    if (spans_generic) {
        LaunchTimer t(prof, ws, st, K_TILE_SCAN, cls_layout[K_TILE_SCAN], cls_algo[K_TILE_SCAN], cls_q[K_TILE_SCAN]);
        launch_tile_scan(st, spans_generic, lds_bytes, pb->d_blobs, pb->d_blob_off, pb->d_span_base, tab(up_qmap_g), n_generic, stack_depth, cand_cap, desc_cap, keys_ptr,
                         hits_ptr, hist_ptr, tile_queue, list_table, facets_generic);
    }
    VQ_HIP(hipGetLastError());
    {
        LaunchTimer t(prof, ws, st, K_MERGE_SPANS, total_span_keys * 8 + total_keys * 8, total_span_keys * 8 + total_keys * 8, nq);
        launch_merge_spans(st, nq, pb->d_blobs, pb->d_blob_off, keys_ptr, reinterpret_cast<unsigned long long*>(pb->d_partial + lay.off_keys));
    }
    VQ_HIP(hipGetLastError());
    VQ_HIP(hipEventRecord(ws.ev_done, st));
    pb->launched = true;
    if (timing_enabled())
        std::fprintf(stderr, "[vq timing] n=%zu compile %.3f ms (dictionary scans %.3f [%zu probes], pass 1 %.3f, unions %.3f [%zu jobs], pass 2 %.3f), range jobs %.3f [%zu], spans generic/simple/and/rich/union %u/%u/%u/%u/%u, pack+launch %.3f ms\n", n,
                     t_compiled - t_start, t_probes - t_start, fuzzy.size(), t_pass1 - t_probes, t_unions - t_pass1, unions.size(), t_compiled - t_ranges,
                     t_ranges - t_unions, ranges.size(), spans_generic, spans_simple, spans_wide, spans_rich, spans_dense + spans_leaf, now_ms() - t_compiled);
    if (timing_enabled())
        std::fprintf(stderr, "[vq timing] pack+launch: span sizing + layout %.3f, blobs + tables %.3f, upload + launches %.3f ms\n", t_layout - t_compiled, t_packed - t_layout, now_ms() - t_packed);
    if (timing_enabled()) {
        uint64_t v[16];
        for (int k = 0; k < 16; ++k) v[k] = g_compile_ns[k].exchange(0);
        if (std::getenv("VQ_TIMING_SUB")) {
            std::fprintf(stderr, "[vq timing] inside 1:n resolve (thread-ms; 6 value-id gather, 7 sort, 8 pairs, 9 order check + layers):");
            for (int k = 6; k < 10; ++k) std::fprintf(stderr, " [%d] %.3f", k, v[k] * 1e-6);
            std::fprintf(stderr, "\n");
        }
        std::fprintf(stderr, "[vq timing] compile thread-ms: total %.3f = dictionary lookups %.3f + 1:n resolve %.3f + 1:n layers %.3f + leaf lists %.3f + rest %.3f; longest request %.3f\n", v[5] * 1e-6,
                     v[0] * 1e-6, v[1] * 1e-6, (v[2] - v[1]) * 1e-6, v[3] * 1e-6, (double(v[5]) - double(v[0]) - double(v[2]) - double(v[3])) * 1e-6, v[4] * 1e-6);
    }
    return pb;
}

std::vector<SuggestEntry> run_suggest(const Index& idx, const vqreq::Request& req) {
    if (!req.suggest) throw VelociError(ERR_INVALID_REQUEST, "only suggest allowed in suggest function");
    VQ_HIP(hipSetDevice(idx.device));
    FuzzyTable fuzzy;
    collect_suggest_probes(idx, req, fuzzy);
    if (!fuzzy.empty()) {
        Workspace& ws = idx.ws[idx.next_ws.fetch_add(1) % kWorkspaces];
        std::unique_lock<std::mutex> lock(ws.mu);
        ws.timed.clear();
        ws.ev_used = 0;
        run_fuzzy_probes(idx, ws, fuzzy, idx.pre_stream ? idx.pre_stream : idx.stream);
    }
    std::vector<SuggestEntry> out;
    for (auto& part : *req.suggest) {
        auto one = suggest_part(idx, part, fuzzy.empty() ? nullptr : &fuzzy);
        out.insert(out.end(), one.begin(), one.end());
    }
    std::stable_sort(out.begin(), out.end(), [](const SuggestEntry& a, const SuggestEntry& b) { return a.text > b.text; });
    std::vector<SuggestEntry> merged;
    for (auto& e : out) {
        if (!merged.empty() && merged.back().text == e.text) {
            if (e.score > merged.back().score) merged.back().score = e.score;
        } else merged.push_back(e);
    }
    std::stable_sort(merged.begin(), merged.end(), [](const SuggestEntry& a, const SuggestEntry& b) { return a.score > b.score; });
    const size_t skip = std::min(req.skip.value_or(0), merged.size());
    merged.erase(merged.begin(), merged.begin() + skip);
    if (req.top && merged.size() > *req.top) merged.resize(*req.top);
    return merged;
}

std::vector<SuggestEntry> run_highlight(const Index& idx, vqreq::RequestSearchPart part) {
    for (auto& t : part.terms) t = vqtext::normalize_text(t);
    VQ_HIP(hipSetDevice(idx.device));
    vqreq::Request probe_req;
    probe_req.suggest = std::vector<vqreq::RequestSearchPart>{part};
    FuzzyTable fuzzy;
    collect_suggest_probes(idx, probe_req, fuzzy);
    if (!fuzzy.empty()) {
        Workspace& ws = idx.ws[idx.next_ws.fetch_add(1) % kWorkspaces];
        std::unique_lock<std::mutex> lock(ws.mu);
        ws.timed.clear();
        ws.ev_used = 0;
        run_fuzzy_probes(idx, ws, fuzzy, idx.pre_stream ? idx.pre_stream : idx.stream);
    }
    std::vector<SuggestEntry> out = highlight_part(idx, part, fuzzy.empty() ? nullptr : &fuzzy);
    std::stable_sort(out.begin(), out.end(), [](const SuggestEntry& a, const SuggestEntry& b) { return a.score > b.score; });
    const size_t skip = std::min(part.skip.value_or(0), out.size());
    out.erase(out.begin(), out.begin() + skip);
    if (part.top && out.size() > *part.top) out.resize(*part.top);
    return out;
}

vqreq::Request page_request_after(const vqreq::Request& R, float score, uint32_t id) {
    vqreq::Request page = R;
    page.top = size_t(kMaxTopK);
    page.skip = 0;
    page.facets.reset();
    uint32_t bits;
    std::memcpy(&bits, &score, 4);
    page.key_upper = (uint64_t(order_f32(bits)) << 32) | id;
    return page;
}

void complete_deep_requests(const Index& idx, const vqreq::Request* const* reqs, size_t n, std::vector<std::unique_ptr<Result>>& results,
                            std::vector<int>& status, std::vector<std::string>& errors) {
    constexpr uint64_t kMaxDeep = 65536;
    for (size_t i = 0; i < n; ++i) {
        if (status[i] != 0 || !results[i] || !results[i]->deep) continue;
        const vqreq::Request& R = *reqs[i];
        Result& out = *results[i];
        out.deep = false;
        const uint64_t top = R.top.value_or(10), skip = R.skip.value_or(0);
        const uint64_t want = top + skip < top ? ~0ull : top + skip;
        std::vector<uint32_t> ids = std::move(out.ids);
        std::vector<float> scores = std::move(out.scores);
        out.ids.clear();
        out.scores.clear();
        if (skip >= out.num_hits) continue;
        const uint64_t reach = std::min<uint64_t>(want, out.num_hits);
        if (reach > kMaxDeep) {
            status[i] = ERR_UNSUPPORTED;
            errors[i] = "unsupported on the MI355X query path: top + skip reaches more than " + std::to_string(kMaxDeep) + " ranked hits";
            results[i].reset();
            continue;
        }
        vqreq::Request page = R;
        page.top = size_t(kMaxTopK);
        page.skip = 0;
        page.facets.reset();
        bool failed = false;
        while (ids.size() < reach && ids.size() % size_t(kMaxTopK) == 0 && !ids.empty()) {
            uint32_t bits;
            std::memcpy(&bits, &scores.back(), 4);
            page.key_upper = (uint64_t(order_f32(bits)) << 32) | ids.back();
            const vqreq::Request* arr[1] = {&page};
            std::vector<std::unique_ptr<Result>> r;
            std::vector<int> st;
// ... 436 lines not shown
```

### veloci_amd/csrc/index.cpp

```cpp
#include <algorithm>
#include <atomic>
#include <chrono>
#include <cstring>
#include <exception>
#include <mutex>
#include <thread>
#include <sys/mman.h>

#include "engine.hpp"
#include "text.hpp"

namespace vq {

const char* const TOKENS_TO_TEXT_ID = ".tokens_to_text_id";
const char* const TO_ANCHOR_ID_SCORE = ".to_anchor_id_score";
const char* const PHRASE_PAIR_TO_ANCHOR = ".phrase_pair_to_anchor";
const char* const VALUE_ID_TO_PARENT = ".value_id_to_parent";
const char* const PARENT_TO_VALUE_ID = ".parent_to_value_id";
const char* const TEXT_ID_TO_ANCHOR = ".text_id_to_anchor";
const char* const ANCHOR_TO_TEXT_ID = ".anchor_to_text_id";
const char* const BOOST_VALID_TO_VALUE = ".boost_valid_to_value";
const char* const TOKEN_VALUES = ".token_values";
const char* const VALUE_ID_TO_ANCHOR = ".value_id_to_anchor";
const char* const TEXTINDEX = ".textindex";
// ... 138 lines not shown
    idx->bitmap_words = ((uint64_t(hi) - idx->bitmap_base + 65535u) / 65536u) * 2048u + 2048u;

    for (auto& [path, f] : b.fst) {
        Dictionary d;
        d.terms = f.terms;
        d.lower_map.reserve(d.terms.size());
        for (uint32_t i = 0; i < d.terms.size(); ++i) d.lower_map[vqtext::to_lower_utf8(d.terms[i])].push_back(i);
        {
            std::vector<uint32_t> off(d.terms.size() + 1, 0u);
            std::vector<uint32_t> raw, low;
            for (uint32_t i = 0; i < d.terms.size(); ++i) {
                for (uint32_t cp : vqtext::decode_utf8(d.terms[i])) {
                    if (cp > 0xFFFFu) d.char_bytes = 4;
                    if (cp == 0x130u) d.low_exact = false;
                    raw.push_back(cp);
                    low.push_back(vqtext::lower_cp(cp));
                }
                off[i + 1] = uint32_t(raw.size());
            }
            auto image = [&](DevBuf& dst, const std::vector<uint32_t>& cps) {
                if (d.char_bytes == 4) {
                    dst.alloc(cps.size() * 4 + 16);
                    dst.upload(cps.data(), cps.size() * 4);
                } else {
                    const std::vector<uint16_t> narrow(cps.begin(), cps.end());
                    dst.alloc(narrow.size() * 2 + 16);
                    dst.upload(narrow.data(), narrow.size() * 2);
                }
            };
            d.d_off.alloc(off.size() * 4 + 16);
            d.d_off.upload(off.data(), off.size() * 4);
            image(d.d_raw, raw);
            image(d.d_low, low);
            idx->device_bytes += d.d_off.bytes + d.d_raw.bytes + d.d_low.bytes;
        }
        idx->dict.emplace(path, std::move(d));
    }

    const size_t nthreads = host_threads();
    auto upload = [&](DevBuf& dst, const void* src, size_t n) {
        const size_t piece = size_t(256) << 20;
        parallel_for((n + piece - 1) / piece, nthreads, [&](size_t i) {
            VQ_HIP(hipSetDevice(device));
            const size_t off = i * piece;
            VQ_HIP(hipMemcpy(dst.as<uint8_t>() + off, static_cast<const uint8_t*>(src) + off, std::min(piece, n - off), hipMemcpyHostToDevice));
        });
    };
    for (const auto& kv : b.postings) {
        const std::string& path = kv.first;
        const HostPostings& p = kv.second;
        PostingStore ps;
        ps.num_tokens = uint32_t(p.offsets.size() - 1);
        ps.start.resize(ps.num_tokens);
        ps.len.resize(ps.num_tokens);
        ps.global_len.resize(ps.num_tokens);
        ps.max_raw.assign(ps.num_tokens, 0);
        std::vector<uint64_t> src_at(ps.num_tokens);
        uint64_t total = 0;
        for (uint32_t t = 0; t < ps.num_tokens; ++t) {
            const uint32_t* rb = p.anchors.data() + p.offsets[t];
            const uint32_t* re = p.anchors.data() + p.offsets[t + 1];
            const uint32_t *sb, *se;
            shard_subrange(rb, re, lo, hi, &sb, &se);
            src_at[t] = uint64_t(sb - p.anchors.data());
            ps.start[t] = total;
            ps.len[t] = uint32_t(se - sb);
            ps.global_len[t] = p.global_lens.empty() ? uint64_t(re - rb) : p.global_lens[t];
            total += (uint64_t(ps.len[t]) + 3u) & ~uint64_t(3);
        }
        uninit_vector<uint32_t> docs(total);
        uninit_vector<uint16_t> scores(total);
        parallel_for(ps.num_tokens, nthreads, [&](size_t t) {
            const uint64_t s0 = ps.start[t], n = ps.len[t], padded = (n + 3u) & ~uint64_t(3);
            std::memcpy(docs.data() + s0, p.anchors.data() + src_at[t], n * 4);
            const uint32_t* sc = p.scores.data() + src_at[t];
            uint16_t most = 0;
            for (uint64_t i = 0; i < n; ++i) {
                const uint16_t h = f32_to_f16_rne(float(sc[i]));
                scores[s0 + i] = h;
                most = std::max(most, h);
            }
            for (uint64_t i = n; i < padded; ++i) {
                docs[s0 + i] = 0xFFFFFFFFu;
                scores[s0 + i] = 0;
            }
            ps.max_raw[t] = most;
        });
        ps.total_padded = total;
        ps.bm_start.assign(ps.num_tokens, -1);
        ps.rd_start.assign(ps.num_tokens, -1);
        {
            const uint64_t range = uint64_t(hi) - lo;
            const uint64_t words = idx->bitmap_words, blocks = words >> (kRankShift - 5);
            std::vector<uint32_t> dense;
            for (uint32_t t = 0; t < ps.num_tokens; ++t)
                if (range >= 65536 && uint64_t(ps.len[t]) * 64 >= range) dense.push_back(t);
            if (!dense.empty()) {
                uninit_vector<uint32_t> bits(words * dense.size());
                uninit_vector<uint32_t> rdir((blocks + 1) * dense.size());
                parallel_for(dense.size(), nthreads, [&](size_t k) {
                    const uint32_t t = dense[k];
                    uint32_t* bw = bits.data() + words * k;
                    uint32_t* rd = rdir.data() + (blocks + 1) * k;
                    std::memset(bw, 0, words * 4);
                    std::memset(rd, 0, (blocks + 1) * 4);
                    const uint32_t* d = docs.data() + ps.start[t];
                    for (uint32_t i = 0; i < ps.len[t]; ++i) {
                        const uint32_t rel = d[i] - idx->bitmap_base;
                        bw[rel >> 5] |= 1u << (rel & 31u);
                        rd[(rel >> kRankShift) + 1] += 1;
                    }
                    for (uint64_t bl = 1; bl <= blocks; ++bl) rd[bl] += rd[bl - 1];
                    ps.bm_start[t] = int64_t(words * k);
                    ps.rd_start[t] = int64_t((blocks + 1) * k);
                });
                ps.bitmaps.alloc(bits.size() * 4 + 16);
                upload(ps.bitmaps, bits.data(), bits.size() * 4);
                ps.rank_dir.alloc(rdir.size() * 4 + 16);
                upload(ps.rank_dir, rdir.data(), rdir.size() * 4);
                idx->device_bytes += ps.bitmaps.bytes + ps.rank_dir.bytes;
            }
        }
        ps.td_start.assign(ps.num_tokens, -1);
        std::vector<uint32_t> tiled;
        {
            const uint64_t range = uint64_t(hi) - lo;
            const uint64_t tiles = (idx->bitmap_words >> (kTileDirShift - 5)) + 3;
            for (uint32_t t = 0; t < ps.num_tokens; ++t) {
                if (range < 65536 || uint64_t(ps.len[t]) * 4096 < range) continue;
                ps.td_start[t] = int64_t(tiled.size() * (tiles + 1));
                tiled.push_back(t);
            }
            std::vector<uint32_t> tdir(tiled.size() * (tiles + 1));
            parallel_for(tiled.size(), nthreads, [&](size_t j) {
                const uint32_t t = tiled[j];
                const uint32_t* d = docs.data() + ps.start[t];
                uint32_t* out = tdir.data() + j * (tiles + 1);
                uint32_t i = 0;
                for (uint64_t k = 0; k <= tiles; ++k) {
                    const uint64_t bound = uint64_t(idx->bitmap_base) + (k << kTileDirShift);
                    while (i < ps.len[t] && d[i] < bound) ++i;
                    out[k] = i;
                }
            });
            if (!tdir.empty()) {
                ps.tile_dir.alloc(tdir.size() * 4 + 16);
                ps.tile_dir.upload(tdir.data(), tdir.size() * 4);
                idx->device_bytes += ps.tile_dir.bytes;
            }
        }
        ps.pk_start.assign(ps.num_tokens, -1);
        ps.ak_start.assign(ps.num_tokens, -1);
        ps.gd_start.assign(ps.num_tokens, -1);
        {
            const uint64_t ptiles = (idx->bitmap_words >> (kProbeTileShift - 5)) + 2;
            uint64_t cov_gran = 0, arr_gran = 0;
            std::vector<uint32_t> gd(tiled.size() * (ptiles + 1));
            std::vector<uint64_t> gran_of(tiled.size());
            std::vector<uint32_t> most_of(tiled.size());
            parallel_for(tiled.size(), nthreads, [&](size_t j) {
                const uint32_t t = tiled[j];
                const uint32_t* d = docs.data() + ps.start[t];
                uint32_t* g = gd.data() + j * (ptiles + 1);
                uint64_t gran = 0;
                uint32_t i = 0, most = 0;
                for (uint64_t k = 0; k <= ptiles; ++k) {
                    g[k] = uint32_t(gran);
                    const uint64_t thi = uint64_t(idx->bitmap_base) + ((k + 1) << kProbeTileShift);
                    const uint32_t i0 = i;
                    while (i < ps.len[t] && d[i] < thi) ++i;
                    const uint32_t n8 = (i - i0 + 7u) / 8u;
                    most = std::max(most, n8);
                    gran += n8;
                }
                gran_of[j] = gran;
                most_of[j] = most;
            });
            for (size_t j = 0; j < tiled.size(); ++j) {
                const uint32_t t = tiled[j];
                ps.gd_start[t] = int64_t(j * (ptiles + 1));
                if (gran_of[j] >= (1ull << 28)) throw VelociError(vqreq::ERR_INVALID_ARGUMENT, "posting list too long for its tile-packed image");
                ps.pk_start[t] = int64_t(cov_gran);
                cov_gran += gran_of[j];
                if (most_of[j] <= 256) {
                    ps.ak_start[t] = int64_t(arr_gran);
                    arr_gran += gran_of[j];
                }
            }
            if (cov_gran) {
                ps.cov32.alloc(cov_gran * 32 + 4096);
                ps.arr16.alloc(arr_gran * 16 + 4096);
                ps.gdir.alloc(gd.size() * 4 + 16);
                ps.gdir.upload(gd.data(), gd.size() * 4);
                idx->device_bytes += ps.cov32.bytes + ps.arr16.bytes + ps.gdir.bytes;
                uninit_vector<uint32_t> cov(cov_gran * 8);
                uninit_vector<uint16_t> arr(arr_gran * 8);
                parallel_for(tiled.size(), nthreads, [&](size_t j) {
                    const uint32_t t = tiled[j];
                    const bool as_array = ps.ak_start[t] >= 0;
                    const uint32_t* d = docs.data() + ps.start[t];
                    const uint16_t* sc = scores.data() + ps.start[t];
                    uint32_t* c = cov.data() + uint64_t(ps.pk_start[t]) * 8;
                    uint16_t* a = as_array ? arr.data() + uint64_t(ps.ak_start[t]) * 8 : nullptr;
                    uint64_t w = 0;
                    uint32_t i = 0;
                    for (uint64_t k = 0; k <= ptiles; ++k) {
                        const uint64_t tlo = uint64_t(idx->bitmap_base) + (k << kProbeTileShift), thi = tlo + (1u << kProbeTileShift);
                        for (; i < ps.len[t] && d[i] < thi; ++i, ++w) {
                            const uint32_t rel = uint32_t(d[i] - tlo);
                            c[w] = rel << 16 | sc[i];
                            if (a) a[w] = uint16_t(rel);
                        }
                        for (; w % 8; ++w) {
                            c[w] = 0xFFFFFFFFu;
                            if (a) a[w] = 0xFFFFu;
                        }
                    }
                });
                upload(ps.cov32, cov.data(), cov.size() * 4);
                upload(ps.arr16, arr.data(), arr.size() * 2);
            }
        }
        ps.docs.alloc(docs.size() * 4 + 16);
        upload(ps.docs, docs.data(), docs.size() * 4);
        ps.scores.alloc(scores.size() * 2 + 16);
        upload(ps.scores, scores.data(), scores.size() * 2);
        idx->device_bytes += ps.docs.bytes + ps.scores.bytes;
        idx->postings.emplace(path, std::move(ps));
    }

    for (auto& [path, k] : b.kv) {
        KVStore s;
        s.key_base = k.key_base;
        s.num_keys = uint32_t(k.offsets.size() - 1);
        s.host_off = k.offsets;
        s.host_values = k.values;
        bool identity_t2t = false;
        if (ends_with(path, TOKENS_TO_TEXT_ID)) {
            std::string ti = path.substr(0, path.size() - std::strlen(TOKENS_TO_TEXT_ID));
            identity_t2t = idx->is_anchor_identity(ti);
        }
        s.list_rows = ends_with(path, TEXT_ID_TO_ANCHOR) || identity_t2t;
        if (identity_t2t) {
            std::string pp = path.substr(0, path.size() - std::strlen(TOKENS_TO_TEXT_ID)) + TO_ANCHOR_ID_SCORE;
            auto bit = b.postings.find(pp);
            if (bit != b.postings.end() && bit->second.offsets.size() == k.offsets.size() && k.key_base == 0) {
                const auto& po = bit->second;
                bool same = po.offsets == k.offsets && po.anchors.size() == k.values.size() &&
                            std::memcmp(po.anchors.data(), k.values.data(), k.values.size() * 4) == 0;
                s.rows_equal_postings = same;
            }
        }
        if (s.list_rows) {
            s.start.resize(s.num_keys);
            s.len.resize(s.num_keys);
            std::vector<uint32_t> vals;
            vals.reserve(k.values.size() + 4);
            std::vector<uint32_t> tmp;
            for (uint32_t r = 0; r < s.num_keys; ++r) {
                const uint32_t* rb = k.values.data() + k.offsets[r];
                const uint32_t* re = k.values.data() + k.offsets[r + 1];
                if (!std::is_sorted(rb, re) || std::adjacent_find(rb, re) != re) {
                    tmp.assign(rb, re);
                    std::sort(tmp.begin(), tmp.end());
                    tmp.erase(std::unique(tmp.begin(), tmp.end()), tmp.end());
                    rb = tmp.data();
                    re = tmp.data() + tmp.size();
                    s.rows_sorted_unique = false;
                }
                const uint32_t *sb, *se;
                shard_subrange(rb, re, lo, hi, &sb, &se);
                s.start[r] = vals.size();
                s.len[r] = uint32_t(se - sb);
                append_padded(vals, sb, se);
            }
            s.values.alloc(vals.size() * 4 + 16);
            s.values.upload(vals.data(), vals.size() * 4);
            idx->device_bytes += s.values.bytes;
            if (ends_with(path, TEXT_ID_TO_ANCHOR)) {
                s.d_row_start.alloc(s.start.size() * 8 + 16);
                s.d_row_start.upload(s.start.data(), s.start.size() * 8);
                s.d_row_len.alloc(s.len.size() * 4 + 16);
                s.d_row_len.upload(s.len.data(), s.len.size() * 4);
                idx->device_bytes += s.d_row_start.bytes + s.d_row_len.bytes;
            }
        }
        if (ends_with(path, TOKENS_TO_TEXT_ID) && !identity_t2t) {
            s.text_csr = true;
            s.d_text_vals.alloc(k.values.size() * 4 + 16);
            s.d_text_vals.upload(k.values.data(), k.values.size() * 4);
            idx->device_bytes += s.d_text_vals.bytes;
        }
        if (ends_with(path, VALUE_ID_TO_PARENT) || ends_with(path, VALUE_ID_TO_ANCHOR)) {
            s.value_csr = true;
            s.d_text_vals.alloc(k.values.size() * 4 + 16);
            s.d_text_vals.upload(k.values.data(), k.values.size() * 4);
            s.d_csr_off.alloc(k.offsets.size() * 8 + 16);
            s.d_csr_off.upload(k.offsets.data(), k.offsets.size() * 8);
            idx->device_bytes += s.d_text_vals.bytes + s.d_csr_off.bytes;
        }
        s.facet_csr = ends_with(path, ANCHOR_TO_TEXT_ID) || (ends_with(path, PARENT_TO_VALUE_ID) && path.find("[]") == std::string::npos);
        if (s.facet_csr) {
            const uint64_t kb = k.key_base, ke = uint64_t(k.key_base) + s.num_keys;
            const uint64_t nb = std::min<uint64_t>(std::max<uint64_t>(kb, lo), ke);
            const uint64_t ne = std::max<uint64_t>(nb, std::min<uint64_t>(ke, hi));
            std::vector<uint64_t> off(ne - nb + 1);
            const uint64_t first = k.offsets[nb - kb];
            for (uint64_t r = nb; r <= ne; ++r) off[r - nb] = k.offsets[r - kb] - first;
            s.csr_off.alloc(off.size() * 8);
            s.csr_off.upload(off.data(), off.size() * 8);
            const uint64_t nvals = k.offsets[ne - kb] - first;
            s.csr_values.alloc(nvals * 4 + 16);
            s.csr_values.upload(k.values.data() + first, nvals * 4);
            idx->device_bytes += s.csr_off.bytes + s.csr_values.bytes;
            s.csr_key_base = uint32_t(nb);
            s.csr_num_keys = uint32_t(ne - nb);
            for (uint64_t e = first; e < first + nvals; ++e) s.csr_max_value = std::max(s.csr_max_value, k.values[e]);
            bool single = true;
            for (size_t r = 0; r + 1 < off.size() && single; ++r) single = off[r + 1] - off[r] <= 1;
            if (single && s.csr_num_keys) {
                std::vector<uint32_t> direct(s.csr_num_keys, 0xFFFFFFFFu);
                for (size_t r = 0; r + 1 < off.size(); ++r)
                    if (off[r + 1] > off[r]) direct[r] = k.values[first + off[r]];
                s.csr_direct.alloc(direct.size() * 4 + 16);
                s.csr_direct.upload(direct.data(), direct.size() * 4);
                idx->device_bytes += s.csr_direct.bytes;
            }
        }
        idx->kv.emplace(path, std::move(s));
    }

    for (auto& [path, p] : b.phrase) {
        PhraseStore s;
        const size_t n = p.t1.size();
        s.keys.reserve(n);
// ... 103 lines not shown
```

### veloci_amd/csrc/kernels.hpp

```cpp
#pragma once
#include <hip/hip_runtime.h>
#include <stddef.h>
#include <stdint.h>

#include "device_types.hpp"

namespace vq {

struct DictProbe {
    uint32_t m, max_d, flags, lm;
    uint16_t query[64];
    uint16_t lquery[64];
};
struct DictProbeW {
    uint32_t m, max_d, flags, lm;
    uint32_t q_off;
    uint32_t lq_off;
    uint32_t pad[2];
};
constexpr uint32_t kDictMaxPattern = 1u << 20;
struct DictMatch {
    uint32_t probe, term;
    uint32_t info;
};

struct UList {
    const uint32_t* docs;
    const void* scores;
    uint32_t len;
    float term_score;
    uint32_t flags, pad;
};
struct RangeJobD {
    uint32_t list_begin, n_lists, anchor_begin, n_anchors, block_begin, pad;
};
struct UTask {
    uint32_t list_begin, n_lists;
    uint32_t span_begin, n_spans;
    uint32_t pivot, pad;
};

struct FacetJob {
    uint32_t hist_off, num_values, top, out_off;
};

size_t tile_scan_lds_bytes(uint32_t n_bitmaps, uint32_t n_lists, uint32_t tile_words, uint32_t stack_depth, uint32_t cand_cap, uint32_t desc_cap, bool queue, uint32_t ml);

void launch_tile_scan(hipStream_t st, uint32_t total_spans, size_t lds_bytes, const uint8_t* blobs, const uint32_t* blob_off, const uint32_t* span_base,
                      const uint32_t* qmap, uint32_t nq, uint32_t stack_depth, uint32_t cand_cap, uint32_t desc_cap, unsigned long long* span_keys, unsigned long long* num_hits, uint32_t* hist, bool queue, uint32_t ml,
                      bool facet_cache = false);
void launch_scan_leaf_f32(hipStream_t st, uint32_t total_spans, const uint8_t* blobs, const uint32_t* blob_off, const uint32_t* span_base, const uint32_t* qmap,
                          uint32_t nq, uint32_t cand_cap, unsigned long long* span_keys, unsigned long long* num_hits, uint32_t* hist);
size_t scan_simple_lds_bytes(uint32_t cand_cap, uint32_t nv, uint32_t n_scatter, bool facet_cache);
uint32_t debug_div100_mismatches();
int debug_facet_select(const uint32_t* hist_host, uint32_t num_values, uint32_t top, uint32_t misalign, uint32_t* out_vals_host, uint32_t* out_counts_host);
void launch_scan_simple(hipStream_t st, bool wide, uint32_t n_scatter, uint32_t total_spans, const uint8_t* blobs, const uint32_t* blob_off, const uint32_t* span_base,
                        const uint32_t* qmap, uint32_t nq, uint32_t cand_cap, unsigned long long* span_keys, unsigned long long* num_hits, uint32_t* hist, bool facet_cache = false);
size_t scan_probe_lds_bytes(uint32_t cand_cap, uint32_t nd);
void launch_scan_probe(hipStream_t st, uint32_t max_nd, uint32_t total_spans, const uint8_t* blobs, const uint32_t* blob_off, const uint32_t* span_base, const uint32_t* qmap,
                       uint32_t nq, uint32_t cand_cap, unsigned long long* span_keys, unsigned long long* num_hits, bool any_and = true, bool any_or = false);
uint32_t scan_ring_consumers(uint32_t max_nd);
uint32_t scan_ring_slots(uint32_t maxnd, uint32_t consumers);
size_t scan_ring_lds_bytes(uint32_t maxnd, uint32_t consumers, uint32_t slots);
void launch_scan_ring(hipStream_t st, uint32_t max_nd, uint32_t grid, const uint8_t* blobs, const uint32_t* blob_off, const uint32_t* qmap, uint32_t nq, uint32_t spans_each,
                      const uint32_t* items, uint32_t total_items, uint32_t* work, unsigned long long* span_keys, unsigned long long* num_hits);
size_t scan_wide_lds_bytes(uint32_t cand_cap, uint32_t n_leaves, uint32_t n_scatter);
void launch_scan_wide(hipStream_t st, uint32_t max_leaves, uint32_t max_scatter, uint32_t total_spans, const uint8_t* blobs, const uint32_t* blob_off, const uint32_t* span_base,
                      const uint32_t* qmap, uint32_t nq, uint32_t cand_cap, unsigned long long* span_keys, unsigned long long* num_hits);
void launch_merge_spans(hipStream_t st, uint32_t nq, const uint8_t* blobs, const uint32_t* blob_off, const unsigned long long* span_keys,
                        unsigned long long* part_keys);
void launch_finalize(hipStream_t st, uint32_t nq, const uint8_t* blobs, const uint32_t* blob_off, const uint8_t* gathered, uint32_t num_shards,
                     size_t shard_stride, const PartialLayout& lay, uint32_t* res_ids, float* res_scores, uint32_t* res_n, unsigned long long* res_hits);
void launch_facet_select(hipStream_t st, uint32_t n_jobs, const FacetJob* jobs, const uint32_t* hist, uint32_t* out_vals, uint32_t* out_counts,
                         uint32_t* out_n);

void launch_range_hits(hipStream_t st, uint32_t n_blocks, uint32_t n_jobs, const UList* ulists, const RangeJobD* jobs, const uint32_t* anchors, unsigned long long* counts);
void launch_union(hipStream_t st, bool write, uint32_t total_spans, const UList* ulists, const UTask* tasks, const uint32_t* span_task, uint32_t* span_cnt,
                  const uint64_t* span_off, uint32_t* out_docs, float* out_vals, uint32_t* task_min);
void launch_scan_union(hipStream_t st, bool with_or, uint32_t total_spans, const uint8_t* blobs, const uint32_t* blob_off, const uint32_t* span_base, const uint32_t* qmap,
                       uint32_t nq, uint32_t cand_cap, unsigned long long* span_keys, unsigned long long* num_hits);
void launch_dict_scan(hipStream_t st, const DictProbe* d_probes, uint32_t probe_base, uint32_t n_probes, const uint32_t* off, const uint16_t* chars, const uint16_t* low_chars,
                      uint32_t num_terms, uint32_t* out_count, uint32_t out_cap, DictMatch* out);
void launch_dict_scan_wide(hipStream_t st, uint32_t char_bytes, const DictProbeW* d_probes, const uint32_t* pool, uint32_t probe_base, uint32_t n_probes, const uint32_t* off,
                           const void* chars, const void* low_chars, uint32_t num_terms, uint32_t* out_count, uint32_t out_cap, DictMatch* out);

struct LocRow {
    uint64_t src, dst;
    uint32_t len, pad;
};
struct LocJob {
    const uint32_t* t2a_vals;
    const uint64_t* t2a_start;
    const uint32_t* t2a_len;
    uint32_t t2a_key_base, t2a_num_keys;
    uint32_t seg_begin, seg_end;
    uint32_t pair_begin, pair_end;
    uint32_t out_off, pad;
};
void launch_loc_gather(hipStream_t st, const LocRow* rows, uint32_t n_rows, const uint32_t* table, uint32_t* gathered);
void launch_loc_expand(hipStream_t st, bool write, const LocJob* jobs, uint32_t n_jobs, const uint32_t* sorted_text_ids, uint32_t n, uint32_t* totals_or_cursors,
                       unsigned long long* pairs);
void launch_loc_compact(hipStream_t st, const LocJob* jobs, uint32_t n_jobs, const unsigned long long* sorted_pairs, uint32_t* out_docs, float* out_vals, uint32_t* out_len);
size_t seg_sort_u32(void* tmp, size_t tmp_bytes, const uint32_t* in, uint32_t* out, uint32_t n, uint32_t nseg, const uint32_t* seg_begin, const uint32_t* seg_end,
                    hipStream_t st);
size_t seg_sort_u64(void* tmp, size_t tmp_bytes, const unsigned long long* in, unsigned long long* out, uint32_t n, uint32_t nseg, const uint32_t* seg_begin,
                    const uint32_t* seg_end, hipStream_t st);

struct B1nJob {
    const uint32_t* boost_present;
    const float* boost_values;
    const uint64_t* to_anchor_off;
    const uint32_t* to_anchor_vals;
    uint32_t boost_key_base, boost_num_keys, to_anchor_key_base, to_anchor_num_keys;
    uint32_t seg_begin, seg_end, out_off, doc_lo, doc_hi, pad;
};
struct B1nResult {
    uint32_t len, total, flags, pad;
};
void launch_b1n_map(hipStream_t st, const B1nJob* jobs, uint32_t n_jobs, const uint32_t* sorted_value_ids, uint32_t* out_docs, float* out_vals, B1nResult* results);

struct ExList {
    const uint32_t* docs;
    const uint16_t* scores;
    uint32_t len;
    float term_score;
};
constexpr uint32_t XP_LEAF = 0, XP_AND = 1, XP_OR = 2;
struct ExOp {
    uint32_t kind, nchild;
    uint32_t a;
    uint32_t b;
};
struct ExQuery {
    uint32_t op_begin, n_ops, list_begin, n_lists, col_begin, n_col;
    uint32_t doc_begin, trace_begin;
};
constexpr uint32_t kExStack = 256;
__host__ __device__ inline uint32_t explain_trace_words(uint32_t n_lists, uint32_t n_ops, uint32_t n_col) { return 3u * (n_lists + n_ops + n_col + 1u); }
void launch_explain(hipStream_t st, uint32_t n_docs, const ExQuery* queries, const uint32_t* doc_query, const uint32_t* docs, const ExOp* ops, const uint16_t* aux,
                    const ExList* lists, const DColBoost* cols, uint32_t* trace);

#ifdef VQ_STAMP
void debug_read_stamps(unsigned long long* out, int reset);
void debug_read_probe_stamps(unsigned long long* out, int reset);
void debug_read_ring_stamps(unsigned long long* out, int reset);
#endif

}
```

### veloci_amd/csrc/scan_probe.hip

```cpp
#include <hip/hip_runtime.h>
#include <hip/hip_fp16.h>

#include "device_types.hpp"
#include "kernel_common.hpp"
#include "kernels.hpp"
#include "probe_common.hpp"

namespace vq {

#ifdef VQ_STAMP
__device__ unsigned long long g_probe_stamp[16];
#define PS_INIT                                                      \
    unsigned long long _st0 = __builtin_amdgcn_s_memtime();          \
    const unsigned long long _t0 = _st0;                             \
    const unsigned long long _r0 = __builtin_amdgcn_s_memrealtime(); \
    unsigned long long _acc[16] = {0};
#define PS_AT(k)                                                \
    {                                                           \
        unsigned long long _st1 = __builtin_amdgcn_s_memtime(); \
        _acc[k] += _st1 - _st0;                                 \
        _st0 = _st1;                                            \
    }
#define PS_COUNT(k) _acc[k] += 1ull;
#define PS_FLUSH                                                                                             \
    _acc[14] = __builtin_amdgcn_s_memtime() - _t0;                        \
    _acc[15] = __builtin_amdgcn_s_memrealtime() - _r0;                \
    if (threadIdx.x == 0) {                                                                                  \
        _Pragma("unroll") for (int _k = 0; _k < 16; ++_k) if (_acc[_k]) atomicAdd(&g_probe_stamp[_k], _acc[_k]); \
    }
void debug_read_probe_stamps(unsigned long long* out, int reset) {
    (void)hipMemcpyFromSymbol(out, HIP_SYMBOL(g_probe_stamp), sizeof(unsigned long long) * 16);
    if (reset) {
        unsigned long long z[16] = {0};
        (void)hipMemcpyToSymbol(HIP_SYMBOL(g_probe_stamp), z, sizeof z);
    }
}
#else
#define PS_INIT
#define PS_AT(k)
#define PS_COUNT(k)
#define PS_FLUSH
#endif

constexpr uint32_t kPMaxR = 2;
constexpr uint32_t kPU = 64 + kPMaxR * 256;
constexpr uint32_t kPR = 128;
constexpr uint32_t kPLdsShape = 8;
constexpr uint32_t kPLdsU = kPLdsShape + 32;
constexpr uint32_t kPLdsR = kPLdsU + kPU;
__host__ __device__ constexpr uint32_t probe_lds_tile(uint32_t nd) { return kPLdsR + (2 + nd) * kPR; }
__host__ __device__ constexpr uint32_t probe_lds_cand(uint32_t nd) { return probe_lds_tile(nd) + nd * (kPTW + kPRk); }
size_t scan_probe_lds_bytes(uint32_t cand_cap, uint32_t nd) { return (size_t)(probe_lds_cand(nd) + 2 * cand_cap) * 4 + 16; }

template <uint32_t ND, uint32_t NA, bool OR = false>
__device__ __forceinline__ void probe_body(const uint8_t* __restrict__ blob, const uint32_t span, const uint32_t q, const uint32_t cand_cap,
                                           unsigned long long* __restrict__ span_keys, unsigned long long* __restrict__ num_hits) {
    extern __shared__ __attribute__((aligned(16))) uint32_t lds[];
    const uint32_t lane = threadIdx.x;
    const VQ_CONST QHeader* H = as_const<QHeader>(blob);
    const VQ_CONST DList* gl = as_const<DList>(blob + H->off_lists);
    const VQ_CONST DOp* gops = as_const<DOp>(blob + H->off_ops);
    const VQ_CONST DProbe* P = as_const<DProbe>(blob + H->off_simple2);
    const uint32_t sflags = H->simple_flags;
    const uint32_t top_k = H->top_k;
    constexpr uint32_t n = ND + 1u;
    constexpr uint32_t NB = ND - NA;
    constexpr uint32_t NB1 = NB ? NB : 1u, NA1 = NA ? NA : 1u;
    PS_INIT

    unsigned long long* thr = reinterpret_cast<unsigned long long*>(lds);
    uint32_t* cand_n = lds + 2;
    uint32_t* sh = lds + kPLdsShape;
    uint32_t* uq = lds + kPLdsU;
    uint32_t* rq = lds + kPLdsR;
    unsigned long long* cand = reinterpret_cast<unsigned long long*>(lds + probe_lds_cand(ND));
    uint32_t* tile = lds + probe_lds_tile(ND);
    uint32_t* rank = tile + ND * kPTW;
    unsigned long long* const gthr = reinterpret_cast<unsigned long long*>(const_cast<uint8_t*>(blob) + offsetof(QHeader, gthr));
    CandState cs{cand, cand_n, thr, cand_cap, gthr};
    cs.upper = H->key_upper;
    uint32_t* const stat = H->stat_off ? lds + 4 : nullptr;
    uint8_t* const pool = H->off_pool ? const_cast<uint8_t*>(blob) + H->off_pool : nullptr;

    const uint32_t* ccov = nullptr;
    const uint32_t* cgdir = nullptr;
    const uint32_t* d_bitmap[NB1];
    const uint32_t* d_rank[NB1];
    const uint16_t* d_arr[NA1];
    const uint32_t* d_agd[NA1];
    {
        const uint32_t ck = (uint32_t)__ffs((int)((sflags >> 8) & 0xFu)) - 1u;
        const uint32_t am = (sflags >> 12) & 0xFu;
        uint32_t role_of[4] = {0u, 0u, 0u, 0u};
        uint32_t ib = 0, ia = NB;
#pragma unroll
        for (uint32_t k = 0; k < n; ++k) {
            const VQ_CONST DList& d = gl[gops[k].list_begin];
            if (k == ck) {
                ccov = P->leaf[k].cov32;
                cgdir = P->leaf[k].gdir;
                if (lane == 0) {
                    sh[kShCts] = __float_as_uint(d.term_score);
                    sh[kShPrunable] = (d.term_score > 0.0f && d.max_raw < 0x7C00u) ? 1u : 0u;
                }
            } else {
                const bool is_arr = ((am >> k) & 1u) != 0u;
                const uint32_t role = is_arr ? ia : ib;
#pragma unroll
                for (uint32_t j = 0; j < NB; ++j)
                    if (!is_arr && j == role) {
                        d_bitmap[j] = d.bitmap;
                        d_rank[j] = d.rank_dir;
                    }
#pragma unroll
                for (uint32_t a = 0; a < NA; ++a)
                    if (is_arr && NB + a == role) {
                        d_arr[a] = P->leaf[k].arr16;
                        d_agd[a] = P->leaf[k].gdir;
                    }
                if (lane == 0) {
                    const uint16_t mr = d.max_raw;
                    sh[kShTs + role] = __float_as_uint(d.term_score);
                    sh[kShVmax + role] = (d.term_score > 0.0f && mr < 0x7C00u) ? __float_as_uint(posting_value(d.term_score, mr)) : 0x7F800000u;
                    reinterpret_cast<unsigned long long*>(sh + kShScores)[role] = is_arr ? (unsigned long long)(uintptr_t)P->leaf[k].cov32 : (unsigned long long)(uintptr_t)d.scores;
                }
                role_of[k] = 1u + role;
                if (is_arr) ++ia;
                else ++ib;
            }
        }
        const KOp root(gops + n);
#pragma unroll
        for (uint32_t j = 0; j < n; ++j) {
            const uint32_t k = OR ? j : root.and_order(j);
            if (lane == 0) sh[kShSrc + j] = k == 0u ? role_of[0] : k == 1u ? role_of[1] : k == 2u ? role_of[2] : role_of[3];
        }
    }

    const uint32_t n_spans = H->n_spans;
    const unsigned long long range = (unsigned long long)(H->doc_hi - H->doc_lo);
    const uint32_t span_lo = span == 0 ? H->doc_lo : ((H->doc_lo + (uint32_t)(range * span / n_spans)) & ~(kPT - 1u));
    const uint32_t span_hi = span + 1 == n_spans ? H->doc_hi : ((H->doc_lo + (uint32_t)(range * (span + 1) / n_spans)) & ~(kPT - 1u));
    const uint32_t bitmap_base = H->bitmap_base;
    const uint32_t keys_base = H->keys_base;

    if (lane == 0) {
        *thr = __hip_atomic_load(gthr, __ATOMIC_RELAXED, __HIP_MEMORY_SCOPE_AGENT);
        *cand_n = 0;
        lds[4] = 0u;
    }
    __syncthreads();
    unsigned long long thr_seen = *thr;
    uint32_t raw_min = 0u;
    constexpr uint32_t kMasks = OR ? (1u << ND) : 1u;
    uint32_t rmin[kMasks];
    auto take_raw_min = [&](const float thr_f) {
        if (OR) {
#pragma unroll
            for (uint32_t m = 0; m < kMasks; ++m) rmin[m] = probe_raw_min<ND>(sh, thr_f, lane, m);
        } else raw_min = probe_raw_min<ND>(sh, thr_f, lane);
    };
    take_raw_min(__uint_as_float(unorder_f32((uint32_t)(thr_seen >> 32))));

    const u32x4 kSent = u32x4{0xFFFFFFFFu, 0xFFFFFFFFu, 0xFFFFFFFFu, 0xFFFFFFFFu};
    const VQ_GLOBAL u32x4* cc4 = as_global(reinterpret_cast<const u32x4*>(ccov));

    uint32_t un = 0, rn = 0;
    uint32_t ucnt = 0;
    unsigned long long hits = 0;
    unsigned long long g_prev = 0ull;

    const uint32_t t_first = (span_lo - bitmap_base) >> kProbeTileShift;
    const uint32_t t_end = span_hi > span_lo ? ((span_hi - 1u - bitmap_base) >> kProbeTileShift) + 1u : t_first;
    uint32_t dir_base = t_first;
    auto load_dir = [&](const uint32_t* g) { return as_global(g)[dir_base + lane < t_end ? dir_base + lane : t_end]; };
    uint32_t dirv = load_dir(cgdir);
    uint32_t adv[NA1];
#pragma unroll
    for (uint32_t a = 0; a < NA; ++a) adv[a] = load_dir(d_agd[a]);
    auto dir_at = [&](const uint32_t v, const uint32_t tt) { return (uint32_t)__builtin_amdgcn_readlane((int)v, (int)(tt - dir_base)); };

    u32x4 wk[ND][kPNV];
    uint32_t rk[NB1];
    u32x4 nid[kPMaxR], cid[kPMaxR];
#pragma unroll
    for (uint32_t r = 0; r < kPMaxR; ++r) nid[r] = cid[r] = kSent;
    uint32_t pf_rounds = 0, pf_v0 = 0, pf_v1 = 0;
    uint32_t na_g0[NA1], na_nv[NA1];
    uint32_t a_g0[NA1], a_cnt[NA1];
#pragma unroll
    for (uint32_t a = 0; a < NA1; ++a) na_g0[a] = na_nv[a] = a_g0[a] = a_cnt[a] = 0u;
    auto issue_tile = [&](const uint32_t tt, const uint32_t g0, const uint32_t g1) {
        pf_rounds = (g1 - g0 + 31u) >> 5;
        pf_v0 = g0 * 2u;
        pf_v1 = g1 * 2u;
        if (OR || pf_rounds) {
#pragma unroll
            for (uint32_t i = 0; i < NB; ++i) {
                const VQ_GLOBAL u32x4* gb = as_global(reinterpret_cast<const u32x4*>(d_bitmap[i] + (size_t)tt * kPTW));
#pragma unroll
                for (uint32_t h = 0; h < kPNV; ++h) wk[i][h] = gb[h * 64u + lane];
                rk[i] = as_global(d_rank[i])[tt * kPRk + lane];
            }
#pragma unroll
            for (uint32_t a = 0; a < NA; ++a) {
                const VQ_GLOBAL u32x4* ga = as_global(reinterpret_cast<const u32x4*>(d_arr[a]) + na_g0[a]);
#pragma unroll
                for (uint32_t h = 0; h < kPNV; ++h)
                    if (h * 64u + lane < na_nv[a]) wk[NB + a][h] = ga[h * 64u + lane];
            }
#pragma unroll
            for (uint32_t r = 0; r < kPMaxR; ++r) {
                const uint32_t v = pf_v0 + r * 64u + lane;
                nid[r] = kSent;
                if (r < pf_rounds && v < pf_v1) nid[r] = cc4[v];
            }
        }
    };

    uint32_t tile_lo = 0;
    uint32_t f_stage = 0;
    uint32_t f_doc = 0, f_idx[ND];
    float f_vc = 0.0f, f_vd[ND];
    uint16_t f_r = 0;
    bool f_alive = false;
#pragma unroll
    for (uint32_t i = 0; i < ND; ++i) {
        f_idx[i] = 0u;
        f_vd[i] = 0.0f;
    }
// ... 13 lines not shown
                }
                probe_lds_fence();
                if (!wballot(pending)) break;
                cand_prune(cs, top_k);
            }
            if (pool && (tiles_since_merge >= 8u || final)) {
                PS_COUNT(13)
                tiles_since_merge = 0;
                probe_pool_merge<true>(cs, top_k, pool, lane);
            }
            const unsigned long long tn = *thr;
            if ((uint32_t)(tn >> 32) != (uint32_t)(thr_seen >> 32)) take_raw_min(__uint_as_float(unorder_f32((uint32_t)(tn >> 32))));
            thr_seen = tn;
        }
    };
    uint32_t f_mask = 0;
    auto sum_of = [&](const ProbeShape<ND>& S, const float vc, const float (&vd)[ND], const uint32_t mask) { return OR ? probe_or_sum<ND>(S, vc, vd, mask) : probe_sum<ND>(S, vc, vd); };
    auto flush_final = [&](const ProbeShape<ND>& S, const bool final) {
        const float score = sum_of(S, f_vc, f_vd, f_mask);
        const unsigned long long key = ((unsigned long long)order_f32(__float_as_uint(score)) << 32) | (unsigned long long)f_doc;
        f_stage = 0;
        PS_COUNT(12)
        push_keys(key, f_alive && key > *thr && key < cs.upper, final);
    };
    auto flush_service = [&](const bool final) {
        const unsigned long long* sptr = reinterpret_cast<const unsigned long long*>(sh + kShScores);
        unsigned long long gp = sptr[0];
        uint32_t gidx = 0u;
        if (f_stage) {
            const ProbeShape<ND> S = probe_shape<ND>(sh);
            const float thr_f = __uint_as_float(unorder_f32((uint32_t)(*thr >> 32)));
            bool last = true;
#pragma unroll
            for (uint32_t i = 0; i < ND; ++i)
                if (f_stage == i + 1u) {
                    f_vd[i] = posting_value(S.ts[i], f_r);
                    if (i + 1u < ND) {
                        constexpr uint32_t zero = 0;
                        f_alive = f_alive && !(sum_of(S, f_vc, f_vd, f_mask) < thr_f);
                        if (stat && lane == 0) *stat += 2u * (uint32_t)__popcll(wballot(f_alive));
                        gp = sptr[i + 1u < ND ? i + 1u : zero];
                        gidx = (f_alive && (!OR || ((f_mask >> (i + 1u < ND ? i + 1u : zero)) & 1u))) ? f_idx[i + 1u < ND ? i + 1u : zero] : 0u;
                        last = false;
                    }
                }
            if (last) flush_final(S, final);
            else ++f_stage;
        } else if (rn >= 64u || (final && rn)) {
            const uint32_t count = rn < 64u ? rn : 64u;
            probe_lds_fence();
            f_alive = lane < count;
            uint32_t raw = 0;
            const uint32_t slot = (rhead + lane) & (kPR - 1u);
            if (f_alive) {
                f_doc = rq[slot];
                raw = rq[kPR + slot];
#pragma unroll
                for (uint32_t i = 0; i < ND; ++i) f_idx[i] = rq[(2u + i) * kPR + slot];
            }
            if (OR) {
                f_mask = 0u;
#pragma unroll
                for (uint32_t i = 0; i < ND; ++i) f_mask |= f_idx[i] != 0xFFFFFFFFu ? 1u << i : 0u;
            }
            f_vc = posting_value(__uint_as_float(sh[kShCts]), (uint16_t)raw);
#pragma unroll
            for (uint32_t i = 0; i < ND; ++i) f_vd[i] = __uint_as_float(sh[kShVmax + i]);
            if (stat && lane == 0) *stat += 2u * count;
            gidx = (f_alive && (!OR || (f_mask & 1u))) ? f_idx[0] : 0u;
            f_stage = 1u;
            rhead = (rhead + count) & (kPR - 1u);
            rn -= count;
        }
        f_r = as_global(reinterpret_cast<const uint16_t*>((uintptr_t)gp))[gidx];
    };
    auto flush_sync = [&]() {
        const ProbeShape<ND> S = probe_shape<ND>(sh);
        probe_lds_fence();
        const uint32_t slot = (rhead + lane) & (kPR - 1u);
        const uint32_t doc = rq[slot];
        const float vc = posting_value(S.cts, (uint16_t)rq[kPR + slot]);
        float vd[ND];
        uint32_t mask = 0;
#pragma unroll
        for (uint32_t i = 0; i < ND; ++i) {
            const uint16_t* sp = reinterpret_cast<const uint16_t*>((uintptr_t) reinterpret_cast<const unsigned long long*>(sh + kShScores)[i]);
            const uint32_t ix = rq[(2u + i) * kPR + slot];
            if (ix != 0xFFFFFFFFu) mask |= 1u << i;
            vd[i] = posting_value(S.ts[i], as_global(sp)[(OR && ix == 0xFFFFFFFFu) ? 0u : ix]);
        }
        if (stat && lane == 0) *stat += 2u * ND * 64u;
        const float score = sum_of(S, vc, vd, mask);
        const unsigned long long key = ((unsigned long long)order_f32(__float_as_uint(score)) << 32) | (unsigned long long)doc;
        rhead = (rhead + 64u) & (kPR - 1u);
        rn -= 64u;
        push_keys(key, key > *thr && key < cs.upper, false);
    };
    auto bitmap_rank = [&](const uint32_t i, const uint32_t rel) {
        const uint32_t g = rel >> kRankShift, wi = (rel >> 5) & 15u, below = (1u << (rel & 31u)) - 1u;
        const int full = (int)((1u << wi) - 1u);
        const uint32_t* tl = tile + i * kPTW;
        uint32_t acc = rank[i * kPRk + g] + (uint32_t)__popc(tl[rel >> 5] & below);
        const u32x4* gw = reinterpret_cast<const u32x4*>(tl + g * 16u);
#pragma unroll
        for (uint32_t v4 = 0; v4 < 4; ++v4) {
            const u32x4 x = gw[v4];
            acc += (uint32_t)__popc(x.x & (uint32_t)__builtin_amdgcn_sbfe(full, v4 * 4u + 0u, 1u));
            acc += (uint32_t)__popc(x.y & (uint32_t)__builtin_amdgcn_sbfe(full, v4 * 4u + 1u, 1u));
            acc += (uint32_t)__popc(x.z & (uint32_t)__builtin_amdgcn_sbfe(full, v4 * 4u + 2u, 1u));
            acc += (uint32_t)__popc(x.w & (uint32_t)__builtin_amdgcn_sbfe(full, v4 * 4u + 3u, 1u));
        }
        return acc;
    };
    auto rank_some = [&](const uint32_t cnt) {
        while (rn + cnt > kPR) flush_sync();
        probe_lds_fence();
        const uint32_t* const uqe = uq + (un - cnt);
        un -= cnt;
        if (NA == 0u && ND == 2u && cnt <= 32u) {
            const uint32_t el = lane & 31u, role = lane >> 5;
            if (el < cnt) {
                const uint32_t e = uqe[el];
                const uint32_t rel = e >> 16;
                const uint32_t slot = (rhead + rn + el) & (kPR - 1u);
                if (role == 0u) {
                    rq[slot] = tile_lo + rel;
                    rq[kPR + slot] = e & 0xFFFFu;
                }
                const bool here = !OR || ((tile[role * kPTW + (rel >> 5)] >> (rel & 31u)) & 1u) != 0u;
                rq[(2u + role) * kPR + slot] = here ? bitmap_rank(role, rel) : 0xFFFFFFFFu;
            }
            rn += cnt;
        } else if (NA == 0u) {
            if (lane < cnt) {
                const uint32_t e = uqe[lane];
                const uint32_t rel = e >> 16;
                const uint32_t slot = (rhead + rn + lane) & (kPR - 1u);
                rq[slot] = tile_lo + rel;
                rq[kPR + slot] = e & 0xFFFFu;
#pragma unroll
                for (uint32_t i = 0; i < NB; ++i) {
                    const bool here = !OR || ((tile[i * kPTW + (rel >> 5)] >> (rel & 31u)) & 1u) != 0u;
                    rq[(2u + i) * kPR + slot] = here ? bitmap_rank(i, rel) : 0xFFFFFFFFu;
                }
            }
            rn += cnt;
        } else {
            uint32_t e = 0xFFFFFFFFu, pos[NA1];
            bool found = lane < cnt;
            if (found) e = uqe[lane];
            const uint32_t rel = e >> 16;
#pragma unroll
            for (uint32_t a = 0; a < NA; ++a) {
                const uint16_t* A = reinterpret_cast<const uint16_t*>(tile + (NB + a) * kPTW);
                uint32_t lo = 0u, len = a_cnt[a];
#ifdef VQ_PROBE_NO_SEARCH
                lo = rel & 7u;
                len = 0u;
#endif
                while (len > 1u) {
                    const uint32_t half = len >> 1;
                    lo = (uint32_t)A[lo + half] <= rel ? lo + half : lo;
                    len -= half;
                }
#ifdef VQ_PROBE_NO_SEARCH
                found = found && a_cnt[a] != 0u && ((uint32_t)A[lo] ^ rel) < 0x2000u;
#else
                found = found && a_cnt[a] != 0u && (uint32_t)A[lo] == rel;
#endif
                pos[a] = lo;
            }
            const unsigned long long fm = wballot(found);
            hits += (unsigned long long)__popcll(fm);
            const bool live = found && (e & 0xFFFFu) >= raw_min;
            const unsigned long long lm = wballot(live);
            if (lm) {
                if (live) {
                    const uint32_t slot = (rhead + rn + (uint32_t)__popcll(lm & ((1ull << lane) - 1ull))) & (kPR - 1u);
                    rq[slot] = tile_lo + rel;
                    rq[kPR + slot] = e & 0xFFFFu;
#pragma unroll
                    for (uint32_t i = 0; i < NB; ++i) rq[(2u + i) * kPR + slot] = bitmap_rank(i, rel);
#pragma unroll
                    for (uint32_t a = 0; a < NA; ++a) rq[(2u + NB + a) * kPR + slot] = (a_g0[a] * 8u + pos[a]) * 2u;
                }
                rn += (uint32_t)__popcll(lm);
            }
        }
    };
    uint32_t lo_rel = 0, width = 0;
    struct ProbeWords {
        uint32_t w[OR ? ND : 1u][4];
    };
    auto probe_read = [&](const u32x4 e4) {
        const uint32_t ee[4] = {e4.x, e4.y, e4.z, e4.w};
        ProbeWords pw;
#pragma unroll
        for (uint32_t c = 0; c < 4; ++c) {
            const uint32_t a = (ee[c] >> 21) & (kPTW - 1u);
            if (OR) {
#pragma unroll
                for (uint32_t i = 0; i < ND; ++i) pw.w[OR ? i : 0u][c] = tile[i * kPTW + a];
            } else {
                pw.w[0][c] = 0xFFFFFFFFu;
                if (NB) {
                    pw.w[0][c] = tile[a];
#pragma unroll
                    for (uint32_t i = 1; i < NB; ++i) pw.w[0][c] &= tile[i * kPTW + a];
                }
            }
        }
        return pw;
    };
    auto probe_eval = [&](const u32x4 e4, const ProbeWords& pw) {
        const uint32_t ee[4] = {e4.x, e4.y, e4.z, e4.w};
        unsigned long long lm[4];
        bool live[4];
#pragma unroll
        for (uint32_t c = 0; c < 4; ++c) {
            const uint32_t rel = ee[c] >> 16;
            const bool in = (rel - lo_rel) < width;
            if (OR) {
                uint32_t mask = 0;
#pragma unroll
                for (uint32_t i = 0; i < ND; ++i) mask |= ((pw.w[OR ? i : 0u][c] >> (rel & 31u)) & 1u) << i;
                uint32_t need = rmin[0];
#pragma unroll
                for (uint32_t m = 1; m < kMasks; ++m) need = mask == m ? rmin[OR ? m : 0u] : need;
                hits += (unsigned long long)__popcll(wballot(in && mask == 0u));
                live[c] = in && (ee[c] & 0xFFFFu) >= need;
                lm[c] = wballot(live[c]);
                continue;
            }
            const bool bit = ((pw.w[0][c] >> (rel & 31u)) & 1u) != 0u;
            const unsigned long long sm = NB ? (wballot(in) & wballot(bit)) : wballot(in);
            if (NA == 0u) {
                const bool strong = (ee[c] & 0xFFFFu) >= raw_min;
                hits += (unsigned long long)__popcll(sm);
                lm[c] = sm & wballot(strong);
                live[c] = in && bit && strong;
            } else {
                lm[c] = sm;
                live[c] = in && bit;
            }
        }
        if (lm[0] | lm[1] | lm[2] | lm[3]) {
#pragma unroll
            for (uint32_t c = 0; c < 4; ++c) {
                if (live[c]) uq[un + (uint32_t)__popcll(lm[c] & ((1ull << lane) - 1ull))] = ee[c];
                un += (uint32_t)__popcll(lm[c]);
            }
        }
    };

    uint32_t t = t_first;
    tile_lo = bitmap_base + (t_first << kProbeTileShift);
    auto next_arrays = [&](const uint32_t tt) {
#pragma unroll
        for (uint32_t a = 0; a < NA; ++a) {
            na_g0[a] = dir_at(adv[a], tt);
            na_nv[a] = dir_at(adv[a], tt + 1u) - na_g0[a];
        }
    };
    if (t < t_end) {
        next_arrays(t);
        issue_tile(t, dir_at(dirv, t), dir_at(dirv, t + 1u));
    }
    PS_AT(0)
    while (t < t_end) {
        PS_COUNT(8)
        __builtin_amdgcn_s_waitcnt(0x0F70);
        __builtin_amdgcn_s_setprio(3);
        const uint32_t rounds = pf_rounds, v0 = pf_v0, v1 = pf_v1;
        if (OR || rounds) {
            if (OR) {
#pragma unroll
                for (uint32_t h = 0; h < kPNV; ++h) {
                    u32x4 u = wk[0][h];
#pragma unroll
                    for (uint32_t i = 1; i < NB; ++i) u |= wk[i][h];
                    ucnt += (uint32_t)__popc(u.x) + (uint32_t)__popc(u.y) + (uint32_t)__popc(u.z) + (uint32_t)__popc(u.w);
                }
            }
#pragma unroll
            for (uint32_t i = 0; i < NB; ++i) {
#pragma unroll
                for (uint32_t h = 0; h < kPNV; ++h) reinterpret_cast<u32x4*>(tile + i * kPTW)[h * 64u + lane] = wk[i][h];
                rank[i * kPRk + lane] = rk[i];
            }
#pragma unroll
            for (uint32_t a = 0; a < NA; ++a) {
#pragma unroll
                for (uint32_t h = 0; h < kPNV; ++h)
                    if (h * 64u < na_nv[a]) reinterpret_cast<u32x4*>(tile + (NB + a) * kPTW)[h * 64u + lane] = wk[NB + a][h];
                a_g0[a] = na_g0[a];
                a_cnt[a] = na_nv[a] * 8u;
            }
#pragma unroll
            for (uint32_t r = 0; r < kPMaxR; ++r) {
                cid[r] = nid[r];
                asm volatile("" : "+v"(cid[r]));
            }
        }
        {
            uint32_t fr = f_r, glo = (uint32_t)g_prev, ghi = (uint32_t)(g_prev >> 32);
            asm volatile("" : "+v"(fr), "+v"(glo), "+v"(ghi), "+v"(dirv));
#pragma unroll
            for (uint32_t a = 0; a < NA; ++a) asm volatile("" : "+v"(adv[a]));
            f_r = (uint16_t)fr;
            g_prev = ((unsigned long long)ghi << 32) | glo;
        }
        PS_AT(1)
        if (lane == 0 && g_prev > *thr) *thr = g_prev;
        const bool more = t + 1u < t_end;
        uint32_t ng0 = 0, ng1 = 0;
        if (more) {
            if (t + 2u - dir_base >= 64u) {
                dir_base = t + 1u;
                dirv = load_dir(cgdir);
#pragma unroll
                for (uint32_t a = 0; a < NA; ++a) adv[a] = load_dir(d_agd[a]);
            }
            ng0 = dir_at(dirv, t + 1u);
            ng1 = dir_at(dirv, t + 2u);
            next_arrays(t + 1u);
        }
        if (f_stage || rn >= 64u) PS_COUNT(11)
        flush_service(false);
        PS_AT(4)
        if (more) issue_tile(t + 1u, ng0, ng1);
        else pf_rounds = 0;
        if (lane == 0) g_prev = __hip_atomic_load(gthr, __ATOMIC_RELAXED, __HIP_MEMORY_SCOPE_AGENT);
        __builtin_amdgcn_s_setprio(0);
        probe_lds_fence();
        {
            const unsigned long long tn = *thr;
            if ((uint32_t)(tn >> 32) != (uint32_t)(thr_seen >> 32)) take_raw_min(__uint_as_float(unorder_f32((uint32_t)(tn >> 32))));
            thr_seen = tn;
            ++tiles_since_merge;
        }
        PS_AT(5)
#ifdef VQ_PROBE_STREAM_ONLY
        hits += (unsigned long long)__popcll(wballot((cid[0].x ^ cid[1].y) == 0x12345u));
        if (rounds && span == 0xFFFFFFFFu) {
#else
        if (rounds) {
#endif
            const uint32_t tile_end = tile_lo + kPT;
            const uint32_t tile_hi = (tile_end > tile_lo && tile_end < span_hi) ? tile_end : span_hi;
            const uint32_t lo_bound = tile_lo > span_lo ? tile_lo : span_lo;
            lo_rel = lo_bound - tile_lo;
            width = tile_hi - lo_bound;
            {
                ProbeWords pw[kPMaxR];
#pragma unroll
                for (uint32_t r = 0; r < kPMaxR; ++r)
                    if (r < rounds) pw[r] = probe_read(cid[r]);
#pragma unroll
                for (uint32_t r = 0; r < kPMaxR; ++r)
                    if (r < rounds) {
                        PS_COUNT(9)
                        probe_eval(cid[r], pw[r]);
                    }
            }
            for (uint32_t r = kPMaxR; r < rounds; ++r) {
                while (un >= kPU - 256u) rank_some(64u);
                const uint32_t v = v0 + r * 64u + lane;
                u32x4 e4 = kSent;
                if (v < v1) e4 = cc4[v];
                PS_COUNT(9)
                const ProbeWords pw = probe_read(e4);
                probe_eval(e4, pw);
            }
            PS_AT(2)
            while (un) {
                PS_COUNT(10)
                rank_some(un < 64u ? un : 64u);
            }
            PS_AT(3)
        }
        ++t;
        tile_lo += kPT;
    }
    while (f_stage || rn) flush_service(true);
    __syncthreads();
    cand_prune(cs, top_k);
    {
        const uint32_t cn = *cand_n;
        unsigned long long* out = span_keys + (size_t)keys_base + (size_t)span * top_k;
        for (uint32_t i = lane; i < top_k; i += 64u) out[i] = i < cn ? cand[i] : 0ull;
    }
    if (OR) {
        uint32_t total;
        (void)wave_excl_scan_u32(ucnt, &total);
        hits += (unsigned long long)total;
    }
    if (lane == 0 && hits) atomicAdd(&num_hits[q], hits);
    if (lane == 0 && H->stat_off && lds[4]) atomicAdd(&num_hits[H->stat_off], (unsigned long long)lds[4]);
    PS_AT(6)
    PS_FLUSH
}

__device__ __forceinline__ void probe_item(const uint32_t* __restrict__ span_base, const uint32_t* __restrict__ qmap, uint32_t nq, uint32_t* q, uint32_t* span) {
    uint32_t lo = 0, hi = nq;
    const uint32_t wg = blockIdx.x;
    while (hi - lo > 1) {
        uint32_t mid = (lo + hi) >> 1;
        if (span_base[mid] <= wg) lo = mid;
        else hi = mid;
    }
    *span = blockIdx.x - span_base[lo];
    *q = qmap[lo];
}

__global__ __launch_bounds__(64) __attribute__((amdgpu_waves_per_eu(3, 8))) void k_scan_probe(const uint8_t* __restrict__ blobs, const uint32_t* __restrict__ blob_off,
                                                                                               const uint32_t* __restrict__ span_base, const uint32_t* __restrict__ qmap, uint32_t nq,
                                                                                               uint32_t cand_cap, unsigned long long* __restrict__ span_keys,
                                                                                               unsigned long long* __restrict__ num_hits) {
    uint32_t q, span;
    probe_item(span_base, qmap, nq, &q, &span);
    const uint8_t* blob = blobs + blob_off[q];
    const uint32_t n = as_const<QHeader>(blob)->simple_n;
    if ((as_const<QHeader>(blob)->simple_flags >> 27) & 1u) return;
    const uint32_t na = (uint32_t)__popc((as_const<QHeader>(blob)->simple_flags >> 12) & 0xFu);
    if (n == 2u) {
        if (na == 0u) probe_body<1, 0>(blob, span, q, cand_cap, span_keys, num_hits);
        else probe_body<1, 1>(blob, span, q, cand_cap, span_keys, num_hits);
    } else if (n == 3u) {
        if (na == 0u) probe_body<2, 0>(blob, span, q, cand_cap, span_keys, num_hits);
        else if (na == 1u) probe_body<2, 1>(blob, span, q, cand_cap, span_keys, num_hits);
        else probe_body<2, 2>(blob, span, q, cand_cap, span_keys, num_hits);
    } else {
        if (na == 0u) probe_body<3, 0>(blob, span, q, cand_cap, span_keys, num_hits);
        else if (na == 1u) probe_body<3, 1>(blob, span, q, cand_cap, span_keys, num_hits);
        else if (na == 2u) probe_body<3, 2>(blob, span, q, cand_cap, span_keys, num_hits);
        else probe_body<3, 3>(blob, span, q, cand_cap, span_keys, num_hits);
    }
}

__global__ __launch_bounds__(64) __attribute__((amdgpu_waves_per_eu(3, 8))) void k_scan_probe_or(const uint8_t* __restrict__ blobs, const uint32_t* __restrict__ blob_off,
                                                                                                  const uint32_t* __restrict__ span_base, const uint32_t* __restrict__ qmap, uint32_t nq,
                                                                                                  uint32_t cand_cap, unsigned long long* __restrict__ span_keys,
                                                                                                  unsigned long long* __restrict__ num_hits) {
    uint32_t q, span;
    probe_item(span_base, qmap, nq, &q, &span);
    const uint8_t* blob = blobs + blob_off[q];
    const uint32_t n = as_const<QHeader>(blob)->simple_n;
    if (!((as_const<QHeader>(blob)->simple_flags >> 27) & 1u)) return;
    if (n == 2u) probe_body<1, 0, true>(blob, span, q, cand_cap, span_keys, num_hits);
    else probe_body<2, 0, true>(blob, span, q, cand_cap, span_keys, num_hits);
}

void launch_scan_probe(hipStream_t st, uint32_t max_nd, uint32_t total_spans, const uint8_t* blobs, const uint32_t* blob_off, const uint32_t* span_base, const uint32_t* qmap,
                       uint32_t nq, uint32_t cand_cap, unsigned long long* span_keys, unsigned long long* num_hits, bool any_and, bool any_or) {
    if (!total_spans) return;
    if (any_and)
        hipLaunchKernelGGL(k_scan_probe, dim3(total_spans), dim3(64), scan_probe_lds_bytes(cand_cap, max_nd), st, blobs, blob_off, span_base, qmap, nq, cand_cap, span_keys, num_hits);
    if (any_or)
        hipLaunchKernelGGL(k_scan_probe_or, dim3(total_spans), dim3(64), scan_probe_lds_bytes(cand_cap, max_nd), st, blobs, blob_off, span_base, qmap, nq, cand_cap, span_keys, num_hits);
}

}
```

Measured before the change: 158,200.

## Split probe kernel per query shape and size LDS per shape

Probe queries are now bucketed by shape (term count and number of array-coded lists), and one specialized kernel is launched per shape instead of a single kernel with runtime dispatch. Each launch sizes its LDS from the nd and na it actually uses, plus a per-query array slot taken from the fullest tile, instead of the worst case. The unranked queue shrinks from 576 to 256 entries, with an on-demand overflow drain replacing the per-round pre-drain. Lower LDS and a raised waves_per_eu hint for small shapes aim at higher occupancy, at the cost of extra kernel launches and extra drain checks.

```diff
diff --git a/veloci_amd/csrc/capi.cpp b/veloci_amd/csrc/capi.cpp
--- a/veloci_amd/csrc/capi.cpp
+++ b/veloci_amd/csrc/capi.cpp
@@ -236,6 +236,11 @@
 const char* vq_last_error(void) { return g_err.c_str(); }
 const char* vq_version(void) { return "veloci_amd 0.3 (gfx950)"; }
 uint32_t vq_debug_div100_mismatches(void) { return vq::debug_div100_mismatches(); }
+uint32_t vq_debug_probe_occupancy(uint32_t shape, uint32_t nd, uint32_t na, uint32_t arr_slot, uint32_t cand_cap, uint32_t* lds_bytes) {
+    const size_t lds = vq::scan_probe_lds_bytes(cand_cap, nd, na, arr_slot);
+    if (lds_bytes) *lds_bytes = uint32_t(lds);
+    return vq::debug_probe_occupancy(shape, lds);
+}
 uint64_t vq_index_speculative_reruns(const vq_index* index) { return index ? index->idx->or_reruns.load() : 0; }
 int vq_debug_facet_select(const uint32_t* hist, uint32_t num_values, uint32_t top, uint32_t misalign, uint32_t* out_values, uint32_t* out_counts) {
     if (!hist || !out_values || !out_counts) return -1;
diff --git a/veloci_amd/csrc/compile.cpp b/veloci_amd/csrc/compile.cpp
--- a/veloci_amd/csrc/compile.cpp
+++ b/veloci_amd/csrc/compile.cpp
@@ -707,6 +707,7 @@
                 h.d_cov32 = ps.cov32.as<uint32_t>() + uint64_t(ps.pk_start[e.tid]) * 8;
                 h.d_gdir = ps.gdir.as<uint32_t>() + ps.gd_start[e.tid];
                 if (ps.ak_start[e.tid] >= 0) h.d_arr16 = ps.arr16.as<uint16_t>() + uint64_t(ps.ak_start[e.tid]) * 8;
+                h.tile_most = ps.tile_most[e.tid];
             }
             uint32_t li = add_list(h);
             info.cover.push_back(li);
@@ -2170,6 +2171,7 @@
                     for (uint32_t k = 0; k < cq.simple_n; ++k) {
                         const HList& l = cq.lists[cq.ops[k].list_begin];
                         cq.probe.leaf[k] = DProbeLeaf{l.d_cov32, l.d_arr16, l.d_gdir};
+                        if ((arr_mask >> k) & 1u) cq.probe_arr_gran = std::max(cq.probe_arr_gran, l.tile_most);
                     }
                 }
                 static const bool ring = std::getenv("VQ_RING") != nullptr && std::atoi(std::getenv("VQ_RING")) != 0;
diff --git a/veloci_amd/csrc/engine.hpp b/veloci_amd/csrc/engine.hpp
--- a/veloci_amd/csrc/engine.hpp
+++ b/veloci_amd/csrc/engine.hpp
@@ -296,6 +296,7 @@
     std::vector<int64_t> pk_start;
     std::vector<int64_t> ak_start;
     std::vector<int64_t> gd_start;
+    std::vector<uint32_t> tile_most;
     DevBuf cov32, arr16, gdir;
 };
 
@@ -500,6 +501,7 @@
     const uint32_t* d_cov32 = nullptr;
     const uint16_t* d_arr16 = nullptr;
     const uint32_t* d_gdir = nullptr;
+    uint32_t tile_most = 0;
     int inline_idx = -1;
     int inline_val_idx = -1;
 };
@@ -573,6 +575,7 @@
     DSimple2 simple2{};
     DWide wide{};
     DProbe probe{};
+    uint32_t probe_arr_gran = 0;
     std::vector<DFacet> facets;
     std::vector<FacetOut> facet_out;
     std::map<std::string, std::vector<std::string>> why_found_terms;
diff --git a/veloci_amd/csrc/exec.cpp b/veloci_amd/csrc/exec.cpp
--- a/veloci_amd/csrc/exec.cpp
+++ b/veloci_amd/csrc/exec.cpp
@@ -1198,9 +1198,10 @@
     const size_t up_qmap_f = up_span_f + tbl;
     const size_t up_span_x = up_qmap_f + tbl;
     const size_t up_qmap_x = up_span_x + tbl;
+    const size_t tbl_p = align_up(size_t(nq + 1 + kProbeShapes) * 4, 256);
     const size_t up_span_p = up_qmap_x + tbl;
-    const size_t up_qmap_p = up_span_p + tbl;
-    const size_t up_qmap_n = up_qmap_p + tbl;
+    const size_t up_qmap_p = up_span_p + tbl_p;
+    const size_t up_qmap_n = up_qmap_p + tbl_p;
     const size_t up_work_n = up_qmap_n + tbl;
     size_t ring_items_max = 0;
     for (size_t i = 0; i < n; ++i)
@@ -1219,8 +1220,20 @@
     bool facets_rich = false;
     uint32_t n_leaf = 0, spans_leaf = 0;
     uint32_t n_xwide = 0, spans_xwide = 0, leaves_xwide = 0, scatter_xwide = 0;
-    uint32_t n_probe = 0, spans_probe = 0, nd_probe = 1;
-    bool probe_any_and = false, probe_any_or = false;
+    struct ProbeClass {
+        uint32_t first = 0, n = 0, spans = 0;
+        uint32_t na_seen = 0, arr_slot = 0;
+    } pcls[kProbeShapes];
+    auto probe_class = [](const CompiledQuery& cq) -> uint32_t {
+        if ((cq.simple_flags >> 27) & 1u) return kProbeOr;
+        const uint32_t nd = cq.simple_n - 1, na = uint32_t(__builtin_popcount((cq.simple_flags >> 12) & 0xFu));
+        return nd <= 1 ? kProbeAnd1 : nd == 2 ? kProbeAnd2A0 + na : kProbeAnd3A0 + na;
+    };
+    auto on_probe = [](const CompiledQuery& cq) {
+        return cq.status == 0 && ((cq.simple_flags >> 25) & 1u) && !((cq.simple_flags >> 26) & 1u) && !((cq.simple_flags >> 19) & 1u) && !((cq.simple_flags >> 24) & 1u) &&
+               !((cq.simple_flags >> 18) & 1u);
+    };
+    bool any_probe = false;
     uint32_t n_ring = 0, items_ring = 0, nd_ring = 1, ring_spans_each = 0;
     uint64_t cls_layout[K_COUNT_] = {}, cls_algo[K_COUNT_] = {}, cls_q[K_COUNT_] = {};
     {
@@ -1253,9 +1266,19 @@
         uint32_t accf = 0, accx = 0;
         uint32_t* sx = reinterpret_cast<uint32_t*>(hup + up_span_x);
         uint32_t* mx = reinterpret_cast<uint32_t*>(hup + up_qmap_x);
-        uint32_t accg = 0, accs = 0, accd = 0, accw = 0, accr = 0, accp = 0;
+        uint32_t accg = 0, accs = 0, accd = 0, accw = 0, accr = 0;
         uint32_t* sp = reinterpret_cast<uint32_t*>(hup + up_span_p);
         uint32_t* mp = reinterpret_cast<uint32_t*>(hup + up_qmap_p);
+        {
+            uint32_t cnt[kProbeShapes] = {};
+            for (size_t i = 0; i < n; ++i)
+                if (on_probe(pb->queries[i])) ++cnt[probe_class(pb->queries[i])];
+            uint32_t at = 0;
+            for (uint32_t c = 0; c < kProbeShapes; ++c) {
+                pcls[c].first = at;
+                at += cnt[c] + 1;
+            }
+        }
         uint32_t* mn = reinterpret_cast<uint32_t*>(hup + up_qmap_n);
         uint32_t ring_max_spans = 0;
         std::vector<uint32_t> ring_ns;
@@ -1305,11 +1328,14 @@
                 items_ring += cq.n_spans;
             } else if ((cq.simple_flags >> 25) & 1u) {
                 kclass = K_SCAN_PROBE;
-                ((cq.simple_flags >> 27) & 1u ? probe_any_or : probe_any_and) = true;
-                nd_probe = std::max<uint32_t>(nd_probe, cq.simple_n - 1);
-                sp[n_probe] = accp;
-                mp[n_probe++] = qi;
-                accp += cq.n_spans;
+                if (!on_probe(cq)) throw VelociError(ERR_DEVICE, "probe query outside the probe tables (internal)");
+                ProbeClass& pc = pcls[probe_class(cq)];
+                pc.na_seen |= 1u << uint32_t(__builtin_popcount((cq.simple_flags >> 12) & 0xFu));
+                pc.arr_slot = std::max(pc.arr_slot, cq.probe_arr_gran * 4u);
+                sp[pc.first + pc.n] = pc.spans;
+                mp[pc.first + pc.n++] = qi;
+                pc.spans += cq.n_spans;
+                any_probe = true;
             } else if (cq.simple_flags && cq.simple_n > 1 && cq.ops.back().kind == OP_AND) {
                 kclass = K_SCAN_AND;
                 scatter_wide = std::max<uint32_t>(scatter_wide, cq.simple_n - uint32_t(__builtin_popcount(cq.simple_flags & 0xFu)));
@@ -1344,8 +1370,7 @@
         spans_leaf = accf;
         sx[n_xwide] = accx;
         spans_xwide = accx;
-        sp[n_probe] = accp;
-        spans_probe = accp;
+        for (const ProbeClass& pc : pcls) sp[pc.first + pc.n] = pc.spans;
         if (n_ring) {
             if (ring_uniform) ring_spans_each = ring_max_spans;
             else {
@@ -1434,9 +1459,17 @@
                          reinterpret_cast<uint32_t*>(dup + up_work_n), keys_ptr, hits_ptr);
     }
     VQ_HIP(hipGetLastError());
-    if (spans_probe) {
+    if (any_probe) {
         LaunchTimer t(prof, ws, st, K_SCAN_PROBE, cls_layout[K_SCAN_PROBE], cls_algo[K_SCAN_PROBE], cls_q[K_SCAN_PROBE]);
-        launch_scan_probe(st, nd_probe, spans_probe, pb->d_blobs, pb->d_blob_off, tab(up_span_p), tab(up_qmap_p), n_probe, cand_cap, keys_ptr, hits_ptr, probe_any_and, probe_any_or);
+        static const bool trace = std::getenv("VQ_PROBE_TRACE") != nullptr;
+        for (uint32_t c = 0; c < kProbeShapes; ++c)
+            if (pcls[c].spans && trace)
+                std::fprintf(stderr, "probe launch: shape %u, %u queries, %u spans, array slot %u words (fullest tile: %u granules), NA seen 0x%x\n", c, pcls[c].n, pcls[c].spans,
+                             pcls[c].arr_slot, pcls[c].arr_slot / 4, pcls[c].na_seen);
+        for (uint32_t c = 0; c < kProbeShapes; ++c)
+            if (pcls[c].spans)
+                launch_scan_probe_shape(st, c, pcls[c].na_seen, pcls[c].arr_slot, pcls[c].spans, pb->d_blobs, pb->d_blob_off, tab(up_span_p) + pcls[c].first, tab(up_qmap_p) + pcls[c].first,
+                                        pcls[c].n, cand_cap, keys_ptr, hits_ptr);
     }
     VQ_HIP(hipGetLastError());
     if (spans_wide) {
diff --git a/veloci_amd/csrc/index.cpp b/veloci_amd/csrc/index.cpp
--- a/veloci_amd/csrc/index.cpp
+++ b/veloci_amd/csrc/index.cpp
@@ -314,6 +314,7 @@
         ps.pk_start.assign(ps.num_tokens, -1);
         ps.ak_start.assign(ps.num_tokens, -1);
         ps.gd_start.assign(ps.num_tokens, -1);
+        ps.tile_most.assign(ps.num_tokens, 0);
         {
             const uint64_t ptiles = (idx->bitmap_words >> (kProbeTileShift - 5)) + 2;
             uint64_t cov_gran = 0, arr_gran = 0;
@@ -343,6 +344,7 @@
                 ps.gd_start[t] = int64_t(j * (ptiles + 1));
                 if (gran_of[j] >= (1ull << 28)) throw VelociError(vqreq::ERR_INVALID_ARGUMENT, "posting list too long for its tile-packed image");
                 ps.pk_start[t] = int64_t(cov_gran);
+                ps.tile_most[t] = most_of[j];
                 cov_gran += gran_of[j];
                 if (most_of[j] <= 256) {
                     ps.ak_start[t] = int64_t(arr_gran);
diff --git a/veloci_amd/csrc/kernels.hpp b/veloci_amd/csrc/kernels.hpp
--- a/veloci_amd/csrc/kernels.hpp
+++ b/veloci_amd/csrc/kernels.hpp
@@ -56,9 +56,11 @@
 int debug_facet_select(const uint32_t* hist_host, uint32_t num_values, uint32_t top, uint32_t misalign, uint32_t* out_vals_host, uint32_t* out_counts_host);
 void launch_scan_simple(hipStream_t st, bool wide, uint32_t n_scatter, uint32_t total_spans, const uint8_t* blobs, const uint32_t* blob_off, const uint32_t* span_base,
                         const uint32_t* qmap, uint32_t nq, uint32_t cand_cap, unsigned long long* span_keys, unsigned long long* num_hits, uint32_t* hist, bool facet_cache = false);
-size_t scan_probe_lds_bytes(uint32_t cand_cap, uint32_t nd);
-void launch_scan_probe(hipStream_t st, uint32_t max_nd, uint32_t total_spans, const uint8_t* blobs, const uint32_t* blob_off, const uint32_t* span_base, const uint32_t* qmap,
-                       uint32_t nq, uint32_t cand_cap, unsigned long long* span_keys, unsigned long long* num_hits, bool any_and = true, bool any_or = false);
+enum : uint32_t { kProbeAnd1 = 0, kProbeAnd2A0, kProbeAnd2A1, kProbeAnd2A2, kProbeAnd3A0, kProbeAnd3A1, kProbeAnd3A2, kProbeAnd3A3, kProbeOr, kProbeShapes };
+size_t scan_probe_lds_bytes(uint32_t cand_cap, uint32_t nd, uint32_t na, uint32_t arr_slot);
+uint32_t debug_probe_occupancy(uint32_t shape, size_t lds_bytes);
+void launch_scan_probe_shape(hipStream_t st, uint32_t shape, uint32_t na_seen, uint32_t arr_slot, uint32_t total_spans, const uint8_t* blobs, const uint32_t* blob_off,
+                             const uint32_t* span_base, const uint32_t* qmap, uint32_t nq, uint32_t cand_cap, unsigned long long* span_keys, unsigned long long* num_hits);
 uint32_t scan_ring_consumers(uint32_t max_nd);
 uint32_t scan_ring_slots(uint32_t maxnd, uint32_t consumers);
 size_t scan_ring_lds_bytes(uint32_t maxnd, uint32_t consumers, uint32_t slots);
diff --git a/veloci_amd/csrc/scan_probe.hip b/veloci_amd/csrc/scan_probe.hip
--- a/veloci_amd/csrc/scan_probe.hip
+++ b/veloci_amd/csrc/scan_probe.hip
@@ -43,17 +43,20 @@
 #endif
 
 constexpr uint32_t kPMaxR = 2;
-constexpr uint32_t kPU = 64 + kPMaxR * 256;
+constexpr uint32_t kPU = 256;
+static_assert(kPU >= 256, "a round of 256 postings must fit the empty queue");
 constexpr uint32_t kPR = 128;
 constexpr uint32_t kPLdsShape = 8;
-constexpr uint32_t kPLdsU = kPLdsShape + 32;
+constexpr uint32_t kPLdsU = kPLdsShape + 24;
 constexpr uint32_t kPLdsR = kPLdsU + kPU;
 __host__ __device__ constexpr uint32_t probe_lds_tile(uint32_t nd) { return kPLdsR + (2 + nd) * kPR; }
-__host__ __device__ constexpr uint32_t probe_lds_cand(uint32_t nd) { return probe_lds_tile(nd) + nd * (kPTW + kPRk); }
-size_t scan_probe_lds_bytes(uint32_t cand_cap, uint32_t nd) { return (size_t)(probe_lds_cand(nd) + 2 * cand_cap) * 4 + 16; }
+__host__ __device__ constexpr uint32_t probe_lds_arr(uint32_t nd, uint32_t nb) { return probe_lds_tile(nd) + nb * (kPTW + kPRk); }
+size_t scan_probe_lds_bytes(uint32_t cand_cap, uint32_t nd, uint32_t na, uint32_t arr_slot) {
+    return (size_t)(probe_lds_arr(nd, nd - na) + na * arr_slot + 2 * cand_cap) * 4 + 16;
+}
 
 template <uint32_t ND, uint32_t NA, bool OR = false>
-__device__ __forceinline__ void probe_body(const uint8_t* __restrict__ blob, const uint32_t span, const uint32_t q, const uint32_t cand_cap,
+__device__ __forceinline__ void probe_body(const uint8_t* __restrict__ blob, const uint32_t span, const uint32_t q, const uint32_t cand_cap, const uint32_t arr_slot,
                                            unsigned long long* __restrict__ span_keys, unsigned long long* __restrict__ num_hits) {
     extern __shared__ __attribute__((aligned(16))) uint32_t lds[];
     const uint32_t lane = threadIdx.x;
@@ -73,9 +76,10 @@
     uint32_t* sh = lds + kPLdsShape;
     uint32_t* uq = lds + kPLdsU;
     uint32_t* rq = lds + kPLdsR;
-    unsigned long long* cand = reinterpret_cast<unsigned long long*>(lds + probe_lds_cand(ND));
     uint32_t* tile = lds + probe_lds_tile(ND);
-    uint32_t* rank = tile + ND * kPTW;
+    uint32_t* rank = tile + NB * kPTW;
+    uint32_t* arr = lds + probe_lds_arr(ND, NB);
+    unsigned long long* cand = reinterpret_cast<unsigned long long*>(arr + NA * arr_slot);
     unsigned long long* const gthr = reinterpret_cast<unsigned long long*>(const_cast<uint8_t*>(blob) + offsetof(QHeader, gthr));
     CandState cs{cand, cand_n, thr, cand_cap, gthr};
     cs.upper = H->key_upper;
@@ -395,7 +399,7 @@
             const uint32_t rel = e >> 16;
 #pragma unroll
             for (uint32_t a = 0; a < NA; ++a) {
-                const uint16_t* A = reinterpret_cast<const uint16_t*>(tile + (NB + a) * kPTW);
+                const uint16_t* A = reinterpret_cast<const uint16_t*>(arr + a * arr_slot);
                 uint32_t lo = 0u, len = a_cnt[a];
 #ifdef VQ_PROBE_NO_SEARCH
                 lo = rel & 7u;
@@ -455,7 +459,7 @@
         }
         return pw;
     };
-    auto probe_eval = [&](const u32x4 e4, const ProbeWords& pw) {
+    auto probe_eval = [&](const u32x4 e4, const ProbeWords& pw, const bool may_overflow) {
         const uint32_t ee[4] = {e4.x, e4.y, e4.z, e4.w};
         unsigned long long lm[4];
         bool live[4];
@@ -488,6 +492,10 @@
             }
         }
         if (lm[0] | lm[1] | lm[2] | lm[3]) {
+            if (may_overflow) {
+                const uint32_t add = (uint32_t)__popcll(lm[0]) + (uint32_t)__popcll(lm[1]) + (uint32_t)__popcll(lm[2]) + (uint32_t)__popcll(lm[3]);
+                while (un + add > kPU) rank_some(un < 64u ? un : 64u);
+            }
 #pragma unroll
             for (uint32_t c = 0; c < 4; ++c) {
                 if (live[c]) uq[un + (uint32_t)__popcll(lm[c] & ((1ull << lane) - 1ull))] = ee[c];
@@ -535,7 +543,7 @@
             for (uint32_t a = 0; a < NA; ++a) {
 #pragma unroll
                 for (uint32_t h = 0; h < kPNV; ++h)
-                    if (h * 64u < na_nv[a]) reinterpret_cast<u32x4*>(tile + (NB + a) * kPTW)[h * 64u + lane] = wk[NB + a][h];
+                    if (h * 64u + lane < na_nv[a]) reinterpret_cast<u32x4*>(arr + a * arr_slot)[h * 64u + lane] = wk[NB + a][h];
                 a_g0[a] = na_g0[a];
                 a_cnt[a] = na_nv[a] * 8u;
             }
@@ -603,17 +611,16 @@
                 for (uint32_t r = 0; r < kPMaxR; ++r)
                     if (r < rounds) {
                         PS_COUNT(9)
-                        probe_eval(cid[r], pw[r]);
+                        probe_eval(cid[r], pw[r], r > 0u);
                     }
             }
             for (uint32_t r = kPMaxR; r < rounds; ++r) {
-                while (un >= kPU - 256u) rank_some(64u);
                 const uint32_t v = v0 + r * 64u + lane;
                 u32x4 e4 = kSent;
                 if (v < v1) e4 = cc4[v];
                 PS_COUNT(9)
                 const ProbeWords pw = probe_read(e4);
-                probe_eval(e4, pw);
+                probe_eval(e4, pw, true);
             }
             PS_AT(2)
             while (un) {
@@ -656,51 +663,78 @@
     *q = qmap[lo];
 }
 
-__global__ __launch_bounds__(64) __attribute__((amdgpu_waves_per_eu(3, 8))) void k_scan_probe(const uint8_t* __restrict__ blobs, const uint32_t* __restrict__ blob_off,
-                                                                                               const uint32_t* __restrict__ span_base, const uint32_t* __restrict__ qmap, uint32_t nq,
-                                                                                               uint32_t cand_cap, unsigned long long* __restrict__ span_keys,
-                                                                                               unsigned long long* __restrict__ num_hits) {
-    uint32_t q, span;
-    probe_item(span_base, qmap, nq, &q, &span);
+#define VQ_PROBE_PARAMS                                                                                                                                       \
+    const uint8_t *__restrict__ blobs, const uint32_t *__restrict__ blob_off, const uint32_t *__restrict__ span_base, const uint32_t *__restrict__ qmap, uint32_t nq, \
+        uint32_t cand_cap, uint32_t arr_slot, unsigned long long *__restrict__ span_keys, unsigned long long *__restrict__ num_hits
+#define VQ_PROBE_ITEM                           \
+    uint32_t q, span;                           \
+    probe_item(span_base, qmap, nq, &q, &span); \
     const uint8_t* blob = blobs + blob_off[q];
-    const uint32_t n = as_const<QHeader>(blob)->simple_n;
-    if ((as_const<QHeader>(blob)->simple_flags >> 27) & 1u) return;
-    const uint32_t na = (uint32_t)__popc((as_const<QHeader>(blob)->simple_flags >> 12) & 0xFu);
-    if (n == 2u) {
-        if (na == 0u) probe_body<1, 0>(blob, span, q, cand_cap, span_keys, num_hits);
-        else probe_body<1, 1>(blob, span, q, cand_cap, span_keys, num_hits);
-    } else if (n == 3u) {
-        if (na == 0u) probe_body<2, 0>(blob, span, q, cand_cap, span_keys, num_hits);
-        else if (na == 1u) probe_body<2, 1>(blob, span, q, cand_cap, span_keys, num_hits);
-        else probe_body<2, 2>(blob, span, q, cand_cap, span_keys, num_hits);
-    } else {
-        if (na == 0u) probe_body<3, 0>(blob, span, q, cand_cap, span_keys, num_hits);
-        else if (na == 1u) probe_body<3, 1>(blob, span, q, cand_cap, span_keys, num_hits);
-        else if (na == 2u) probe_body<3, 2>(blob, span, q, cand_cap, span_keys, num_hits);
-        else probe_body<3, 3>(blob, span, q, cand_cap, span_keys, num_hits);
-    }
-}
-
-__global__ __launch_bounds__(64) __attribute__((amdgpu_waves_per_eu(3, 8))) void k_scan_probe_or(const uint8_t* __restrict__ blobs, const uint32_t* __restrict__ blob_off,
-                                                                                                  const uint32_t* __restrict__ span_base, const uint32_t* __restrict__ qmap, uint32_t nq,
-                                                                                                  uint32_t cand_cap, unsigned long long* __restrict__ span_keys,
-                                                                                                  unsigned long long* __restrict__ num_hits) {
-    uint32_t q, span;
-    probe_item(span_base, qmap, nq, &q, &span);
-    const uint8_t* blob = blobs + blob_off[q];
-    const uint32_t n = as_const<QHeader>(blob)->simple_n;
-    if (!((as_const<QHeader>(blob)->simple_flags >> 27) & 1u)) return;
-    if (n == 2u) probe_body<1, 0, true>(blob, span, q, cand_cap, span_keys, num_hits);
-    else probe_body<2, 0, true>(blob, span, q, cand_cap, span_keys, num_hits);
-}
-
-void launch_scan_probe(hipStream_t st, uint32_t max_nd, uint32_t total_spans, const uint8_t* blobs, const uint32_t* blob_off, const uint32_t* span_base, const uint32_t* qmap,
-                       uint32_t nq, uint32_t cand_cap, unsigned long long* span_keys, unsigned long long* num_hits, bool any_and, bool any_or) {
+#ifndef VQ_PROBE_WAVES
+#define VQ_PROBE_WAVES 4
+#endif
+#define VQ_PROBE_KERNEL(waves) __global__ __launch_bounds__(64) __attribute__((amdgpu_waves_per_eu(waves, 8))) void
+
+VQ_PROBE_KERNEL(VQ_PROBE_WAVES) k_scan_probe_1(VQ_PROBE_PARAMS) {
+    VQ_PROBE_ITEM
+    if (((as_const<QHeader>(blob)->simple_flags >> 12) & 0xFu) == 0u) probe_body<1, 0>(blob, span, q, cand_cap, arr_slot, span_keys, num_hits);
+    else probe_body<1, 1>(blob, span, q, cand_cap, arr_slot, span_keys, num_hits);
+}
+VQ_PROBE_KERNEL(VQ_PROBE_WAVES) k_scan_probe_2_0(VQ_PROBE_PARAMS) {
+    VQ_PROBE_ITEM
+    probe_body<2, 0>(blob, span, q, cand_cap, arr_slot, span_keys, num_hits);
+}
+VQ_PROBE_KERNEL(VQ_PROBE_WAVES) k_scan_probe_2_1(VQ_PROBE_PARAMS) {
+    VQ_PROBE_ITEM
+    probe_body<2, 1>(blob, span, q, cand_cap, arr_slot, span_keys, num_hits);
+}
+VQ_PROBE_KERNEL(VQ_PROBE_WAVES) k_scan_probe_2_2(VQ_PROBE_PARAMS) {
+    VQ_PROBE_ITEM
+    probe_body<2, 2>(blob, span, q, cand_cap, arr_slot, span_keys, num_hits);
+}
+VQ_PROBE_KERNEL(3) k_scan_probe_3_0(VQ_PROBE_PARAMS) {
+    VQ_PROBE_ITEM
+    probe_body<3, 0>(blob, span, q, cand_cap, arr_slot, span_keys, num_hits);
+}
+VQ_PROBE_KERNEL(3) k_scan_probe_3_1(VQ_PROBE_PARAMS) {
+    VQ_PROBE_ITEM
+    probe_body<3, 1>(blob, span, q, cand_cap, arr_slot, span_keys, num_hits);
+}
+VQ_PROBE_KERNEL(3) k_scan_probe_3_2(VQ_PROBE_PARAMS) {
+    VQ_PROBE_ITEM
+    probe_body<3, 2>(blob, span, q, cand_cap, arr_slot, span_keys, num_hits);
+}
+VQ_PROBE_KERNEL(3) k_scan_probe_3_3(VQ_PROBE_PARAMS) {
+    VQ_PROBE_ITEM
+    probe_body<3, 3>(blob, span, q, cand_cap, arr_slot, span_keys, num_hits);
+}
+
+VQ_PROBE_KERNEL(3) k_scan_probe_or(VQ_PROBE_PARAMS) {
+    VQ_PROBE_ITEM
+    if (as_const<QHeader>(blob)->simple_n == 2u) probe_body<1, 0, true>(blob, span, q, cand_cap, arr_slot, span_keys, num_hits);
+    else probe_body<2, 0, true>(blob, span, q, cand_cap, arr_slot, span_keys, num_hits);
+}
+
+static auto* probe_kernel(uint32_t shape) {
+    return shape == kProbeAnd1 ? k_scan_probe_1 : shape == kProbeAnd2A0 ? k_scan_probe_2_0 : shape == kProbeAnd2A1 ? k_scan_probe_2_1 : shape == kProbeAnd2A2 ? k_scan_probe_2_2 :
+           shape == kProbeAnd3A0 ? k_scan_probe_3_0 : shape == kProbeAnd3A1 ? k_scan_probe_3_1 : shape == kProbeAnd3A2 ? k_scan_probe_3_2 : shape == kProbeAnd3A3 ? k_scan_probe_3_3 :
+                                                                                                                                                                    k_scan_probe_or;
+}
+
+uint32_t debug_probe_occupancy(uint32_t shape, size_t lds_bytes) {
+    int n = 0;
+    if (shape >= kProbeShapes || hipOccupancyMaxActiveBlocksPerMultiprocessor(&n, probe_kernel(shape), 64, lds_bytes) != hipSuccess || n < 0) return 0;
+    return (uint32_t)n;
+}
+
+void launch_scan_probe_shape(hipStream_t st, uint32_t shape, uint32_t na_seen, uint32_t arr_slot, uint32_t total_spans, const uint8_t* blobs, const uint32_t* blob_off,
+                             const uint32_t* span_base, const uint32_t* qmap, uint32_t nq, uint32_t cand_cap, unsigned long long* span_keys, unsigned long long* num_hits) {
     if (!total_spans) return;
-    if (any_and)
-        hipLaunchKernelGGL(k_scan_probe, dim3(total_spans), dim3(64), scan_probe_lds_bytes(cand_cap, max_nd), st, blobs, blob_off, span_base, qmap, nq, cand_cap, span_keys, num_hits);
-    if (any_or)
-        hipLaunchKernelGGL(k_scan_probe_or, dim3(total_spans), dim3(64), scan_probe_lds_bytes(cand_cap, max_nd), st, blobs, blob_off, span_base, qmap, nq, cand_cap, span_keys, num_hits);
-}
-
-}
+    const uint32_t nd = shape == kProbeAnd1 ? 1u : (shape >= kProbeAnd3A0 && shape <= kProbeAnd3A3) ? 3u : 2u;
+    size_t lds = 0;
+    for (uint32_t na = 0; na <= nd; ++na)
+        if ((na_seen >> na) & 1u) lds = std::max(lds, scan_probe_lds_bytes(cand_cap, nd, na, arr_slot));
+    hipLaunchKernelGGL(probe_kernel(shape), dim3(total_spans), dim3(64), lds, st, blobs, blob_off, span_base, qmap, nq, cand_cap, arr_slot, span_keys, num_hits);
+}
+
+}
```

After: 165,200 (median of 6 runs). 1.04x the previous value.
